# Lakonik/SSDNeRF

Hardware: NVIDIA H100
Metric: rays/sec (128^2 render) & DDIM triplanes/sec (higher is better)
Workload: dtype fp16 tensor-core UNet (fp32 accumulate), fp32 renderer

## Files before the change

### ssdnerf_b200/csrc/conv_row2.cu

```cuda
#include "common.cuh"
#include "tc_common.cuh"
#include "conv_row_epilogue.cuh"
#include "../../include/ssdnerf_b200.h"
#include <cuda_fp16.h>

namespace ssdnerf {
using namespace tc;

constexpr int kRwThreads = 384;
constexpr int kRwRowSlot = 17 * 1024;
constexpr int kRwBSlot = kRwN * 128;
constexpr int kRwRows = 6, kRwBStages = 6;
constexpr int kGnMaxC = 384;
constexpr size_t kRwSmem = (size_t)kRwRows * kRwRowSlot + (size_t)kRwBStages * kRwBSlot + 1024  + 256  +
                           256  + 512 ;

struct ConvRowParams {
    uint32_t B, H;
    const __half* x1; uint32_t C1;
    const __half* x2; uint32_t C2;
    long long xs1[3], xs2[3];
    const float2* coef;
    const float* bias;
    const __half* residual;
    __half* out;
    float* qstats;
};

template <bool GN>
__global__ void __launch_bounds__(kRwThreads, 1)
k_conv_row2(const __grid_constant__ CUtensorMap mapB, const ConvRowParams p) {
    extern __shared__ uint8_t smem_raw[];
    uint8_t* smem = reinterpret_cast<uint8_t*>(((uintptr_t)smem_raw + 1023) & ~(uintptr_t)1023);
    uint8_t* sR = smem;
    uint8_t* sB = smem + kRwRows * kRwRowSlot;
    uint64_t* fullR = reinterpret_cast<uint64_t*>(sB + kRwBStages * kRwBSlot);
    uint64_t* emptyR = fullR + kRwRows;
    uint64_t* fullB = emptyR + kRwRows;
    uint64_t* emptyB = fullB + kRwBStages;
    float* qacc = reinterpret_cast<float*>(reinterpret_cast<uint8_t*>(fullR) + 256);
    float* sbias = qacc + 64;

    const int warp = threadIdx.x >> 5, lane = threadIdx.x & 31, wg = warp >> 2;
    const uint32_t tiles_per_img = p.H / 2, total_tiles = p.B * tiles_per_img;
    const uint32_t kc1 = p.C1 / 64, KC = (p.C1 + p.C2) / 64;
    const uint32_t tile0 = blockIdx.x, tstep = gridDim.x;
    const uint32_t my_tiles = tile0 < total_tiles ? (total_tiles - tile0 + tstep - 1) / tstep : 0;

    if (threadIdx.x == 0) {
        prefetch_tmap(&mapB);
        for (int i = 0; i < kRwRows; ++i) { mbar_init(&fullR[i], 4); mbar_init(&emptyR[i], 8); }
        for (int i = 0; i < kRwBStages; ++i) { mbar_init(&fullB[i], 1); mbar_init(&emptyB[i], 8); }
        fence_mbar_init();
    }
    for (int i = threadIdx.x; i < 64; i += kRwThreads) qacc[i] = 0.0f;
    for (int i = threadIdx.x; i < kRwN; i += kRwThreads) sbias[i] = p.bias ? __ldg(p.bias + i) : 0.0f;
    __syncthreads();
    pdl_trigger();
    pdl_wait();

    if (wg == 2) {
        setmaxnreg_dec<120>();
        const uint32_t lt = threadIdx.x - 256u;
        const uint32_t c8 = lt & 7u, p0 = lt >> 3;
        const uint32_t C = p.C1 + p.C2;
        uint32_t idx = 0;
        for (uint32_t tile = tile0; tile < total_tiles; tile += tstep) {
            const uint32_t b = tile / tiles_per_img, y0 = (tile - b * tiles_per_img) * 2;
            for (uint32_t j = 0; j < KC; ++j) {
                const bool first = j < kc1;
                const __half* src = first ? p.x1 : p.x2;
                const long long xs0 = first ? p.xs1[0] : p.xs2[0], xs1 = first ? p.xs1[1] : p.xs2[1], xs2 = first ? p.xs1[2] : p.xs2[2];
                const uint32_t cl = (first ? j : j - kc1) * 64u + c8 * 8u;
                float ca[8], cb[8];
                if (GN) {
                    const float4* cp = reinterpret_cast<const float4*>(p.coef + (size_t)b * C + j * 64u + c8 * 8u);
#pragma unroll
                    for (int k = 0; k < 4; ++k) {
                        const float4 t = __ldg(cp + k);
                        ca[2 * k] = 0.5f * t.x; cb[2 * k] = 0.5f * t.y; ca[2 * k + 1] = 0.5f * t.z; cb[2 * k + 1] = 0.5f * t.w;
                    }
                }
                for (uint32_t r = 0; r < 4; ++r) {
                    const int y = (int)(y0 + r) - 1;
                    const bool row_ok = y >= 0 && y < (int)p.H;
                    const __half* rowp = src + (long long)b * xs2 + (long long)(row_ok ? y : 0) * xs1 + cl;
                    uint4 v[9];
#pragma unroll
                    for (int n = 0; n < 9; ++n) {
                        const int x = (int)(p0 + 16u * n) - 1;
                        v[n] = (row_ok && (unsigned)x < (unsigned)kRwW) ? __ldg(reinterpret_cast<const uint4*>(rowp + (long long)x * xs0))
                                                                       : make_uint4(0, 0, 0, 0);
                    }
                    const uint32_t slot = idx % kRwRows;
                    mbar_wait(&emptyR[slot], ((idx / kRwRows) & 1u) ^ 1u);
                    const uint32_t dst = smem_u32(sR + slot * kRwRowSlot);
#pragma unroll
                    for (int n = 0; n < 9; ++n) {
                        const uint32_t px = p0 + 16u * n;
                        if (px >= 130u) continue;
                        uint4 o = v[n];
                        if (GN) {
                            const bool ok = row_ok && (unsigned)((int)px - 1) < (unsigned)kRwW;
                            const __half2* h = reinterpret_cast<const __half2*>(&v[n]);
                            uint32_t* ow = reinterpret_cast<uint32_t*>(&o);
#pragma unroll
                            for (int k = 0; k < 4; ++k) {
                                const float2 tt = __half22float2(h[k]);
                                const __half2 hh = __floats2half2_rn(fmaf(tt.x, ca[2 * k], cb[2 * k]), fmaf(tt.y, ca[2 * k + 1], cb[2 * k + 1]));
                                uint32_t hv = *reinterpret_cast<const uint32_t*>(&hh), tv;
                                asm("tanh.approx.f16x2 %0, %1;" : "=r"(tv) : "r"(hv));
                                const __half2 yy = __hfma2(hh, *reinterpret_cast<const __half2*>(&tv), hh);
                                ow[k] = ok ? *reinterpret_cast<const uint32_t*>(&yy) : 0u;
                            }
                        }
                        sts128(dst + px * 128u + ((c8 ^ (px & 7u)) << 4), o);
                    }
                    __syncwarp();
                    if (lane == 0) mbar_arrive(&fullR[slot]);
                    ++idx;
                }
            }
        }
    } else {
        setmaxnreg_inc<192>();
        const uint32_t a = (uint32_t)wg, wq = (uint32_t)warp & 3u, cq = (uint32_t)lane & 3u;
        const uint32_t steps_per_tile = KC * 9u, total_steps = my_tiles * steps_per_tile;
        auto issue_w = [&](uint32_t L) {
            const uint32_t s = L % kRwBStages;
            if (L >= (uint32_t)kRwBStages) mbar_wait(&emptyB[s], ((L / kRwBStages) - 1u) & 1u);
            mbar_expect_tx(&fullB[s], (uint32_t)kRwBSlot);
            const uint32_t rem = L % steps_per_tile;
            tma_load_4d(sB + s * kRwBSlot, &mapB, &fullB[s], (int)((rem / 9u) * 64u), 0, (int)(rem % 9u), 0);
        };
        if (threadIdx.x == 0)
            for (uint32_t L = 0; L < total_steps && L < (uint32_t)kRwBStages; ++L) issue_w(L);
        auto release_row = [&](uint32_t ring) { if (lane == 0) mbar_arrive(&emptyR[ring % kRwRows]); };
        uint32_t m = 0, ridx = 0;
        const uint32_t lrow = wq * 16u + ((uint32_t)lane & 15u);
        const uint32_t lk = (uint32_t)lane >> 4;
        for (uint32_t tile = tile0; tile < total_tiles; tile += tstep) {
            const uint32_t b = tile / tiles_per_img, y0 = (tile - b * tiles_per_img) * 2;
            float acc0[64], acc1[64];
#pragma unroll
            for (int i = 0; i < 64; ++i) { acc0[i] = 0.0f; acc1[i] = 0.0f; }
            for (uint32_t j = 0; j < KC; ++j) {
                const uint32_t unused = ridx + (a == 0 ? 3u : 0u);
                if (a == 1) { mbar_wait(&fullR[unused % kRwRows], (unused / kRwRows) & 1u); release_row(unused); }
                for (uint32_t ky = 0; ky < 3; ++ky) {
                    const uint32_t ring = ridx + ky + a;
                    mbar_wait(&fullR[ring % kRwRows], (ring / kRwRows) & 1u);
                    const uint32_t rowS = smem_u32(sR + (ring % kRwRows) * kRwRowSlot);
                    for (uint32_t kx = 0; kx < 3; ++kx) {
                        const uint32_t sb = m % kRwBStages;
                        uint32_t af[2][4][4];
#pragma unroll
                        for (uint32_t h = 0; h < 2; ++h) {
                            const uint32_t px = 64u * h + lrow + kx;
#pragma unroll
                            for (uint32_t k = 0; k < 4; ++k) ldmatrix_x4(rowS + px * 128u + (((2u * k + lk) ^ (px & 7u)) << 4), af[h][k]);
                        }
                        if (kx == 2) release_row(ring);
                        mbar_wait(&fullB[sb], (m / kRwBStages) & 1u);
                        const uint64_t b_desc = make_desc_sw128(smem_u32(sB + sb * kRwBSlot));
                        wgmma_fence();
                        fence_regs(acc0); fence_regs(acc1);
#pragma unroll
                        for (uint32_t k = 0; k < 4; ++k) {
                            wgmma_rs_n128(acc0, af[0][k], b_desc + 2 * k, 1u);
                            wgmma_rs_n128(acc1, af[1][k], b_desc + 2 * k, 1u);
                        }
                        wgmma_commit();
                        wgmma_wait<0>();
                        fence_regs(acc0); fence_regs(acc1);
                        if (lane == 0) mbar_arrive(&emptyB[sb]);
                        if (threadIdx.x == 0 && m >= 1 && m - 1 + kRwBStages < total_steps) issue_w(m - 1 + kRwBStages);
                        ++m;
                    }
                }
                if (a == 0) { mbar_wait(&fullR[unused % kRwRows], (unused / kRwRows) & 1u); release_row(unused); }
                ridx += 4;
            }
            const size_t pix0 = ((size_t)b * p.H + y0 + a) * kRwW;
#pragma unroll
            for (int i = 0; i < 16; ++i) {
                const uint32_t ch = 8u * i + 2u * cq;
                const float b0 = sbias[ch], b1 = sbias[ch + 1];
                float su = 0.0f, sq = 0.0f;
#pragma unroll
                for (int h = 0; h < 2; ++h) {
#pragma unroll
                    for (int hh = 0; hh < 2; ++hh) {
                        const size_t o = (pix0 + 64u * h + wq * 16u + ((uint32_t)lane >> 2) + 8u * hh) * kRwN + ch;
                        float v0 = (h ? acc1 : acc0)[4 * i + 2 * hh] + b0, v1 = (h ? acc1 : acc0)[4 * i + 2 * hh + 1] + b1;
                        if (p.residual) { const float2 r = __half22float2(*reinterpret_cast<const __half2*>(p.residual + o)); v0 += r.x; v1 += r.y; }
                        *reinterpret_cast<__half2*>(p.out + o) = __floats2half2_rn(v0, v1);
                        su += v0 + v1; sq = fmaf(v0, v0, fmaf(v1, v1, sq));
                    }
                }
                if (p.qstats) {
                    frag_quad_reduce(su, sq);
                    if ((lane & ~2) == 0) { float* qa = qacc + (2 * i + (lane >> 1)) * 2; atomicAdd(qa, su); atomicAdd(qa + 1, sq); }
                }
            }
            if (p.qstats) {
                asm volatile("bar.sync 1, 256;" ::: "memory");
                if (threadIdx.x < 64) {
                    const float val = qacc[threadIdx.x];
                    if (val != 0.0f) atomicAdd(p.qstats + (size_t)b * 64 + threadIdx.x, val);
                    qacc[threadIdx.x] = 0.0f;
                }
                asm volatile("bar.sync 1, 256;" ::: "memory");
            }
        }
    }
    __syncthreads();
}

__global__ void k_gn_coef(const float* __restrict__ q1, uint32_t C1, const float* __restrict__ q2, uint32_t C2, uint32_t HW,
                          const float* __restrict__ gamma, const float* __restrict__ beta, const float* __restrict__ scale_shift,
                          long long ss_batch_stride, float eps, float2* __restrict__ coef) {
    pdl_trigger();
    pdl_wait();
    __shared__ float2 s_mr[32];
    const uint32_t b = blockIdx.x, C = C1 + C2, cpg = C / 32u;
    const float inv_n = 1.0f / ((float)HW * (float)cpg);
    if (threadIdx.x < 32u) {
        const uint32_t q1n = C1 / 4, q2n = C2 / 4, nq = cpg / 4;
        float sm = 0.0f, sq = 0.0f;
        for (uint32_t i = 0; i < nq; ++i) {
            const uint32_t qi = threadIdx.x * nq + i;
            const float2 t = __ldg(reinterpret_cast<const float2*>(qi < q1n ? q1 + ((size_t)b * q1n + qi) * 2 : q2 + ((size_t)b * q2n + (qi - q1n)) * 2));
            sm += t.x; sq += t.y;
        }
        const float mean = sm * inv_n;
        s_mr[threadIdx.x] = make_float2(mean, rsqrtf(fmaxf(sq * inv_n - mean * mean, 0.0f) + eps));
    }
    __syncthreads();
    const float* ss = scale_shift ? scale_shift + (size_t)b * ss_batch_stride : nullptr;
    for (uint32_t c = threadIdx.x; c < C; c += blockDim.x) {
        const float2 mr = s_mr[c / cpg];
        const float ak = mr.y * __ldg(gamma + c);
        const float bk = __ldg(beta + c) - mr.x * ak;
        const float sc = ss ? 1.0f + __ldg(ss + c) : 1.0f, sh = ss ? __ldg(ss + C + c) : 0.0f;
        coef[(size_t)b * C + c] = make_float2(ak * sc, fmaf(bk, sc, sh));
    }
}

int make_map_4d_box(CUtensorMap* m, const void* base, uint64_t K, uint64_t e1, uint64_t e2, uint64_t e3, uint64_t s1, uint64_t s2, uint64_t s3,
                    uint32_t x1, uint32_t x2, uint32_t x3);

template <bool GN>
static int launch_row2(const CUtensorMap& mB, const ConvRowParams& p, int sms, cudaStream_t stream) {
    static DeviceOnce attr;
    if (attr.first()) {
        SSDNERF_CUDA_OK(cudaFuncSetAttribute(k_conv_row2<GN>, cudaFuncAttributeMaxDynamicSharedMemorySize, (int)kRwSmem));
    }
    const uint32_t total = p.B * (p.H / 2);
    SSDNERF_CUDA_OK(launch_pdl(k_conv_row2<GN>, dim3(total < (uint32_t)sms ? total : (uint32_t)sms), dim3(kRwThreads), kRwSmem, stream, mB, p));
    SSDNERF_LAUNCH_OK();
    return 0;
}

int conv_row2_launch(const ssdnerf_gemm_args* a, int sms, cudaStream_t stream) {
    if (((uintptr_t)a->a1 & 15u) || ((a->a1_strides[0] | a->a1_strides[1] | a->a1_strides[2]) & 15u) ||
        (a->a2 && (((uintptr_t)a->a2 & 15u) || ((a->a2_strides[0] | a->a2_strides[1] | a->a2_strides[2]) & 15u))) ||
        ((uintptr_t)a->out & 3u) || ((uintptr_t)a->residual & 3u))
        return set_error_msg(SSDNERF_ERR_ARG, "gemm: row-pair convolution needs 16-byte aligned inputs and strides, 4-byte aligned output / residual");
    ConvRowParams p{};
    p.B = a->d3; p.H = a->d2;
    p.x1 = (const __half*)a->a1; p.C1 = a->k1;
    p.x2 = (const __half*)a->a2; p.C2 = a->a2 ? a->k2 : 0;
    for (int i = 0; i < 3; ++i) { p.xs1[i] = (long long)(a->a1_strides[i] / 2); p.xs2[i] = a->a2 ? (long long)(a->a2_strides[i] / 2) : 0; }
    p.bias = a->bias_n; p.residual = (const __half*)a->residual; p.out = (__half*)a->out; p.qstats = a->qstats;
    const uint64_t ktot = (uint64_t)a->k1 + (a->a2 ? a->k2 : 0);
    CUtensorMap mB;
    if (int e = make_map_4d_box(&mB, a->b, ktot, a->n_rows_b ? a->n_rows_b : a->n, a->bx2 ? a->bx2 : 1, a->bx3 ? a->bx3 : 1, a->b_strides[0],
                                a->b_strides[1], a->b_strides[2], kRwN, 1, 1)) return e;
    return launch_row2<false>(mB, p, sms, stream);
}

}

using namespace ssdnerf;

extern "C" int ssdnerf_conv3x3_gn_f16(const ssdnerf_conv_gn_args* a, void* stream_) {
    cudaStream_t stream = (cudaStream_t)stream_;
    if (!a || !a->x1 || !a->q1 || !a->gamma || !a->beta || !a->w || !a->out || !a->coef_workspace)
        return set_error_msg(SSDNERF_ERR_ARG, "conv3x3_gn: x1, q1, gamma, beta, w, out and coef_workspace are required");
    if (a->B == 0 || a->H == 0) return 0;
    if (a->H % 2) return set_error_msg(SSDNERF_ERR_ARG, "conv3x3_gn: H must be even (tiles are row pairs)");
    if (a->C1 == 0 || a->C1 % 64 || a->C2 % 64 || (a->x2 && !a->q2)) return set_error_msg(SSDNERF_ERR_ARG, "conv3x3_gn: channel counts must be multiples of 64; x2 needs q2");
    const uint32_t C = a->C1 + (a->x2 ? a->C2 : 0);
    if (C > (uint32_t)kGnMaxC || (C / 32) % 4) return set_error_msg(SSDNERF_ERR_ARG, "conv3x3_gn: at most 384 input channels, channels per group a multiple of 4");
    if (a->w_rows < 128) return set_error_msg(SSDNERF_ERR_ARG, "conv3x3_gn: packed weight needs >= 128 rows per tap");
    if (((uintptr_t)a->x1 | (uintptr_t)a->x2 | (uintptr_t)a->out | (uintptr_t)a->residual | (uintptr_t)a->w | (uintptr_t)a->coef_workspace) & 15u)
        return set_error_msg(SSDNERF_ERR_ARG, "conv3x3_gn: tensors must be 16-byte aligned");
    ConvRowParams p{};
    p.B = a->B; p.H = a->H; p.x1 = (const __half*)a->x1; p.C1 = a->C1; p.x2 = (const __half*)a->x2; p.C2 = a->x2 ? a->C2 : 0;
    p.xs1[0] = p.C1; p.xs1[1] = (long long)kRwW * p.C1; p.xs1[2] = (long long)p.H * kRwW * p.C1;
    p.xs2[0] = p.C2; p.xs2[1] = (long long)kRwW * p.C2; p.xs2[2] = (long long)p.H * kRwW * p.C2;
    p.coef = (const float2*)a->coef_workspace; p.bias = a->bias; p.residual = (const __half*)a->residual; p.out = (__half*)a->out; p.qstats = a->qstats;
    int dev = 0, sms = 0;
    SSDNERF_CUDA_OK(cudaGetDevice(&dev));
    SSDNERF_CUDA_OK(cudaDeviceGetAttribute(&sms, cudaDevAttrMultiProcessorCount, dev));
    SSDNERF_CUDA_OK(launch_pdl(k_gn_coef, dim3(a->B), dim3(128), 0, stream, a->q1, a->C1, a->x2 ? a->q2 : (const float*)nullptr, p.C2, a->H * 128u,
                               a->gamma, a->beta, a->scale_shift, a->ss_batch_stride, a->eps, (float2*)a->coef_workspace));
    SSDNERF_LAUNCH_OK();
    CUtensorMap mB;
    if (int e = make_map_4d_box(&mB, a->w, C, a->w_rows, 9, 1, (uint64_t)C * 2, (uint64_t)a->w_rows * C * 2, (uint64_t)9 * a->w_rows * C * 2,
                                kRwN, 1, 1)) return e;
    return launch_row2<true>(mB, p, sms, stream);
}
```

### ssdnerf_b200/csrc/conv_row_epilogue.cuh

```cuda
#pragma once
#include "common.cuh"

namespace ssdnerf {

constexpr int kRwW = 128, kRwN = 128;

__device__ __forceinline__ void frag_quad_reduce(float& su, float& sq) {
    su += __shfl_xor_sync(0xffffffffu, su, 1); sq += __shfl_xor_sync(0xffffffffu, sq, 1);
#pragma unroll
    for (int m = 4; m <= 16; m <<= 1) { su += __shfl_xor_sync(0xffffffffu, su, m); sq += __shfl_xor_sync(0xffffffffu, sq, m); }
}

}
```

### ssdnerf_b200/csrc/gemm_tc.cu

```cuda
#include "common.cuh"
#include "tc_common.cuh"
#include "conv_row_epilogue.cuh"
#include "../../include/ssdnerf_b200.h"
#include <cuda_fp16.h>
#include <cstdio>

namespace ssdnerf {
using namespace tc;

constexpr int kGemmThreads = 384;
constexpr int kMaxBiasN = 2048;
constexpr int kBM = 128, kBK = 64;
constexpr int kABytes = kBM * kBK * 2;

struct GemmParams {
    uint32_t b1, b2, b3;
    uint32_t d1, d2, d3;
    uint32_t T1, T2, T3;
    uint32_t tiles_n;
    uint32_t taps;
    int8_t tap_ox[9], tap_oy[9];
    uint32_t a_stride;
    uint32_t kc1, kc2;
    uint32_t n_valid;
    uint32_t b_batched;
    uint32_t vec2;
    float alpha;
    const float* bias_n;
    const __half* residual;
    void* out;
    uint32_t out_f32;
    long long so1, so2, so3;
    float* qstats;
    uint32_t stats_hw;
    unsigned long long* prof;
};

template <int BN, int CL>
struct GemmCfg {
    static constexpr int kBBytes = BN * kBK * 2;
    static constexpr int kBoxRowsB = BN / CL;
    static constexpr int kStageBytes = kABytes + kBBytes;
    static constexpr int kStages = (192 * 1024 / kStageBytes) > 8 ? 8 : (192 * 1024 / kStageBytes);
    static constexpr size_t kSmem = (size_t)kStages * kStageBytes + 1024  + 256  + 1024  +
                                    kMaxBiasN * 4 ;
};

template <int BN, int CL>
__global__ void __launch_bounds__(kGemmThreads, 1)
k_gemm_tc(const __grid_constant__ CUtensorMap mapA1, const __grid_constant__ CUtensorMap mapA2,
          const __grid_constant__ CUtensorMap mapB, const GemmParams p) {
    using Cfg = GemmCfg<BN, CL>;
    extern __shared__ uint8_t smem_raw[];
    uint8_t* smem = reinterpret_cast<uint8_t*>(((uintptr_t)smem_raw + 1023) & ~(uintptr_t)1023);
    uint8_t* sA = smem;
    uint8_t* sB = smem + Cfg::kStages * kABytes;
    uint64_t* full = reinterpret_cast<uint64_t*>(smem + Cfg::kStages * Cfg::kStageBytes);
    uint64_t* empty = full + Cfg::kStages;
    float* qacc = reinterpret_cast<float*>(smem + Cfg::kStages * Cfg::kStageBytes + 256);
    float* sbias = qacc + 256;

    const int warp = threadIdx.x >> 5, lane = threadIdx.x & 31, wg = warp >> 2;
    const uint32_t tiles_m = p.T1 * p.T2 * p.T3;
    const uint32_t sup_m = (tiles_m + CL - 1) / CL;
    const uint32_t total_tiles = sup_m * p.tiles_n;
    const uint32_t iters = p.taps * (p.kc1 + p.kc2);
    const uint32_t crank = (CL > 1) ? cluster_ctarank() : 0u;
    const uint32_t tile0 = (CL > 1) ? cluster_id_x() : blockIdx.x;
    const uint32_t tile_step = (CL > 1) ? num_clusters_x() : gridDim.x;
    constexpr uint16_t kMask = (uint16_t)((1u << CL) - 1u);

    if (threadIdx.x == 0) {
        prefetch_tmap(&mapA1); prefetch_tmap(&mapA2); prefetch_tmap(&mapB);
        for (int i = 0; i < Cfg::kStages; ++i) { mbar_init(&full[i], 1); mbar_init(&empty[i], 8 * CL); }
        fence_mbar_init();
    }
    for (int i = threadIdx.x; i < BN; i += kGemmThreads) qacc[i] = 0.0f;
    if (p.bias_n) for (uint32_t i = threadIdx.x; i < p.n_valid; i += kGemmThreads) sbias[i] = __ldg(p.bias_n + i);
    __syncthreads();
    if (CL > 1) cluster_sync_all();
    pdl_trigger();
    pdl_wait();

    if (wg == 0) {
        setmaxnreg_dec<40>();
        if (threadIdx.x == 0) {
            uint32_t stage = 0, phase = 0;
            long long pw = 0; const long long pt0 = clock64();
            for (uint32_t tile = tile0; tile < total_tiles; tile += tile_step) {
                const uint32_t m_tile = (tile % sup_m) * CL + crank, n_tile = tile / sup_m;
                const uint32_t t1 = m_tile % p.T1, t2 = (m_tile / p.T1) % p.T2, t3 = m_tile / (p.T1 * p.T2);
                for (uint32_t tap = 0; tap < p.taps; ++tap) {
                    const int ox = p.tap_ox[tap], oy = p.tap_oy[tap];
                    for (uint32_t j = 0; j < p.kc1 + p.kc2; ++j) {
                        if (p.prof) { const long long c = clock64(); mbar_wait(&empty[stage], phase ^ 1); pw += clock64() - c; }
                        else mbar_wait(&empty[stage], phase ^ 1);
                        const bool first = j < p.kc1;
                        const int ak = (int)((first ? j : j - p.kc1) * kBK), a1 = (int)(t1 * p.b1 * p.a_stride) + ox, a2 = (int)(t2 * p.b2 * p.a_stride) + oy, a3 = (int)(t3 * p.b3);
                        mbar_expect_tx(&full[stage], (uint32_t)Cfg::kStageBytes);
                        tma_load_4d(sA + stage * kABytes, first ? &mapA1 : &mapA2, &full[stage], ak, a1, a2, a3);
                        if (CL == 1) {
                            tma_load_4d(sB + stage * Cfg::kBBytes, &mapB, &full[stage], (int)(j * kBK), (int)(n_tile * BN),
                                        p.b_batched ? (int)t2 : (int)tap, p.b_batched ? (int)t3 : 0);
                        } else {
                            tma_load_4d_mc(sB + stage * Cfg::kBBytes + crank * Cfg::kBoxRowsB * 128, &mapB, &full[stage], (int)(j * kBK),
                                           (int)(n_tile * BN + crank * Cfg::kBoxRowsB), (int)tap, 0, kMask);
                        }
                        if (++stage == Cfg::kStages) { stage = 0; phase ^= 1; }
                    }
                }
            }
            if (p.prof) { atomicAdd(p.prof + 0, (unsigned long long)pw); atomicAdd(p.prof + 1, (unsigned long long)(clock64() - pt0)); }
        }
    } else {
        setmaxnreg_inc<232>();
        const uint32_t cw = (uint32_t)wg - 1u;
        const uint32_t wq = (uint32_t)warp & 3u;
        const uint32_t rbase = cw * 64u + wq * 16u + ((uint32_t)lane >> 2);
        const uint32_t cq = (uint32_t)lane & 3u;
        uint32_t stage = 0, phase = 0;
        long long wf = 0; const long long ct0 = clock64();
        float acc[BN / 2];
        auto release = [&](uint32_t s) {
            if (lane == 0) {
                if (CL == 1) mbar_arrive(&empty[s]);
                else for (uint32_t r = 0; r < (uint32_t)CL; ++r) mbar_arrive_cluster(mapa_u32(smem_u32(&empty[s]), r));
            }
        };
        for (uint32_t tile = tile0; tile < total_tiles; tile += tile_step) {
            const uint32_t m_tile = (tile % sup_m) * CL + crank, n_tile = tile / sup_m;
            const uint32_t t1 = m_tile % p.T1, t2 = (m_tile / p.T1) % p.T2, t3 = m_tile / (p.T1 * p.T2);
#pragma unroll
            for (int i = 0; i < BN / 2; ++i) acc[i] = 0.0f;
            uint32_t prev = 0;
            for (uint32_t it = 0; it < iters; ++it) {
                if (p.prof && cw == 0) { const long long c = clock64(); mbar_wait(&full[stage], phase); wf += clock64() - c; }
                else mbar_wait(&full[stage], phase);
                const uint64_t a_desc = make_desc_sw128(smem_u32(sA + stage * kABytes + cw * 64 * 128));
                const uint64_t b_desc = make_desc_sw128(smem_u32(sB + stage * Cfg::kBBytes));
                wgmma_fence();
                fence_regs(acc);
#pragma unroll
                for (uint32_t k = 0; k < kBK / 16; ++k) {
                    if constexpr (BN == 256) wgmma_ss_n256(acc, a_desc + 2 * k, b_desc + 2 * k, 1u);
                    else if constexpr (BN == 128) wgmma_ss_n128(acc, a_desc + 2 * k, b_desc + 2 * k, 1u);
                    else wgmma_ss_n64(acc, a_desc + 2 * k, b_desc + 2 * k, 1u);
                }
                wgmma_commit();
                fence_regs(acc);
                wgmma_wait<1>();
                if (it > 0) release(prev);
                prev = stage;
                if (++stage == Cfg::kStages) { stage = 0; phase ^= 1; }
            }
            wgmma_wait<0>();
            fence_regs(acc);
            if (iters > 0) release(prev);

            long long off[2]; bool rok[2];
#pragma unroll
            for (int h = 0; h < 2; ++h) {
                const uint32_t row = rbase + 8u * h;
                const uint32_t i1 = row % p.b1, i2 = (row / p.b1) % p.b2, i3 = row / (p.b1 * p.b2);
                const uint32_t g1 = t1 * p.b1 + i1, g2 = t2 * p.b2 + i2, g3 = t3 * p.b3 + i3;
                rok[h] = m_tile < tiles_m && g1 < p.d1 && g2 < p.d2 && g3 < p.d3;
                off[h] = (long long)g1 * p.so1 + (long long)g2 * p.so2 + (long long)g3 * p.so3 + (long long)n_tile * BN;
            }
            uint32_t slot = 0, img0 = 0;
            if (p.qstats) {
                const uint32_t r0 = cw * 64u;
                const uint32_t j1 = r0 % p.b1, j3 = r0 / (p.b1 * p.b2);
                img0 = p.stats_hw ? (t1 * p.b1) / p.stats_hw : t3 * p.b3;
                slot = ((p.stats_hw ? (t1 * p.b1 + j1) / p.stats_hw : t3 * p.b3 + j3) - img0) & 1u;
            }
#pragma unroll
            for (int i = 0; i < BN / 8; ++i) {
                const uint32_t c0 = 8u * i + 2u * cq;
                const uint32_t ncol = n_tile * BN + c0;
                const bool okc0 = ncol < p.n_valid, okc1 = ncol + 1 < p.n_valid;
                float su = 0.0f, sq = 0.0f;
#pragma unroll
                for (int h = 0; h < 2; ++h) {
                    float v0 = acc[4 * i + 2 * h] * p.alpha, v1 = acc[4 * i + 2 * h + 1] * p.alpha;
                    if (!rok[h] || !okc0) continue;
                    if (p.bias_n) { v0 += sbias[ncol]; if (okc1) v1 += sbias[ncol + 1]; }
                    const long long o = off[h] + c0;
                    if (p.residual) {
                        if (p.vec2 && okc1) {
                            const float2 r = __half22float2(*reinterpret_cast<const __half2*>(p.residual + o));
                            v0 += r.x; v1 += r.y;
                        } else {
                            v0 += __half2float(p.residual[o]);
                            if (okc1) v1 += __half2float(p.residual[o + 1]);
                        }
                    }
                    if (p.out_f32) {
                        float* op = reinterpret_cast<float*>(p.out) + o;
                        if (p.vec2 && okc1) *reinterpret_cast<float2*>(op) = make_float2(v0, v1);
                        else { op[0] = v0; if (okc1) op[1] = v1; }
                    } else {
                        __half* op = reinterpret_cast<__half*>(p.out) + o;
                        if (p.vec2 && okc1) *reinterpret_cast<__half2*>(op) = __floats2half2_rn(v0, v1);
                        else { op[0] = __float2half_rn(v0); if (okc1) op[1] = __float2half_rn(v1); }
                    }
                    if (!okc1) v1 = 0.0f;
                    su += v0 + v1; sq = fmaf(v0, v0, fmaf(v1, v1, sq));
                }
                if (p.qstats) {
                    frag_quad_reduce(su, sq);
                    if ((lane & ~2) == 0) {
                        float* qa = qacc + (slot * (BN / 4) + 2 * i + (lane >> 1)) * 2;
                        atomicAdd(qa, su); atomicAdd(qa + 1, sq);
                    }
                }
            }
            if (p.qstats) {
                asm volatile("bar.sync 1, 256;" ::: "memory");
                const uint32_t et = threadIdx.x - 128;
                const uint32_t nq = p.n_valid / 4;
                for (uint32_t i = et; i < (uint32_t)BN; i += 256) {
                    const float val = qacc[i];
                    const uint32_t sl = i / (BN / 2), qd = (i % (BN / 2)) >> 1, st = i & 1u;
                    const uint32_t gq = n_tile * (BN / 4) + qd;
                    if (val != 0.0f && gq < nq) atomicAdd(p.qstats + ((size_t)(img0 + sl) * nq + gq) * 2 + st, val);
                    qacc[i] = 0.0f;
                }
                asm volatile("bar.sync 1, 256;" ::: "memory");
            }
        }
        if (p.prof && threadIdx.x == 128) { atomicAdd(p.prof + 2, (unsigned long long)wf); atomicAdd(p.prof + 4, (unsigned long long)(clock64() - ct0)); }
    }
    __syncthreads();
    if (CL > 1) cluster_sync_all();
}

typedef CUresult (*PFN_encodeTiled)(CUtensorMap*, CUtensorMapDataType, cuuint32_t, void*, const cuuint64_t*, const cuuint64_t*,
                                    const cuuint32_t*, const cuuint32_t*, CUtensorMapInterleave, CUtensorMapSwizzle,
                                    CUtensorMapL2promotion, CUtensorMapFloatOOBfill);

static PFN_encodeTiled get_encode() {
    static PFN_encodeTiled fn = nullptr;
    if (!fn) {
        void* p = nullptr;
        cudaDriverEntryPointQueryResult qres;
        if (cudaGetDriverEntryPoint("cuTensorMapEncodeTiled", &p, cudaEnableDefault, &qres) != cudaSuccess || !p) return nullptr;
        fn = (PFN_encodeTiled)p;
    }
    return fn;
}

static int make_map_4d(CUtensorMap* m, const void* base, uint64_t K, uint64_t e1, uint64_t e2, uint64_t e3, uint64_t s1, uint64_t s2,
                       uint64_t s3, uint32_t x1, uint32_t x2, uint32_t x3, uint32_t trav = 1) {
    PFN_encodeTiled enc = get_encode();
    if (!enc) return set_error_msg(SSDNERF_ERR_CUDA, "cuTensorMapEncodeTiled entry point not found");
    if (((uintptr_t)base & 15u) || (s1 & 15u) || (s2 & 15u) || (s3 & 15u))
        return set_error_msg(SSDNERF_ERR_ARG, "gemm: TMA operands need 16-byte aligned base and strides");
    cuuint64_t dims[4] = {K, e1, e2, e3};
    cuuint64_t strides[3] = {s1, s2, s3};
    cuuint32_t box[4] = {64, x1 * trav, x2 * trav, x3};
    cuuint32_t estr[4] = {1, trav, trav, 1};
    const CUresult r = enc(m, CU_TENSOR_MAP_DATA_TYPE_FLOAT16, 4, const_cast<void*>(base), dims, strides, box, estr,
                           CU_TENSOR_MAP_INTERLEAVE_NONE, CU_TENSOR_MAP_SWIZZLE_128B, CU_TENSOR_MAP_L2_PROMOTION_L2_256B,
                           CU_TENSOR_MAP_FLOAT_OOB_FILL_NONE);
    if (r != CUDA_SUCCESS) {
        char buf[200];
        snprintf(buf, sizeof(buf), "cuTensorMapEncodeTiled failed (%d): dims {%llu,%llu,%llu,%llu} box {64,%u,%u,%u}", (int)r,
                 (unsigned long long)K, (unsigned long long)e1, (unsigned long long)e2, (unsigned long long)e3, x1, x2, x3);
        return set_error_msg(SSDNERF_ERR_CUDA, buf);
    }
    return 0;
}

int make_map_4d_box(CUtensorMap* m, const void* base, uint64_t K, uint64_t e1, uint64_t e2, uint64_t e3, uint64_t s1, uint64_t s2, uint64_t s3,
                    uint32_t x1, uint32_t x2, uint32_t x3) {
    return make_map_4d(m, base, K, e1, e2, e3, s1, s2, s3, x1, x2, x3);
}
int conv_row2_launch(const ssdnerf_gemm_args* a, int sms, cudaStream_t stream);

template <int BN, int CL>
static int launch_gemm(const CUtensorMap& mA1, const CUtensorMap& mA2, const CUtensorMap& mB, const GemmParams& p, int sms,
                       cudaStream_t stream) {
    using Cfg = GemmCfg<BN, CL>;
    static DeviceOnce attr;
    if (attr.first()) {
        SSDNERF_CUDA_OK(cudaFuncSetAttribute(k_gemm_tc<BN, CL>, cudaFuncAttributeMaxDynamicSharedMemorySize, (int)Cfg::kSmem));
    }
    const uint32_t tiles_m = p.T1 * p.T2 * p.T3;
    const uint32_t total = ((tiles_m + CL - 1) / CL) * p.tiles_n;
    cudaLaunchConfig_t cfg{};
    cfg.blockDim = dim3(kGemmThreads);
    cfg.dynamicSmemBytes = Cfg::kSmem;
    cfg.stream = stream;
    cudaLaunchAttribute at[2];
    at[0].id = cudaLaunchAttributeClusterDimension;
    at[0].val.clusterDim.x = CL; at[0].val.clusterDim.y = 1; at[0].val.clusterDim.z = 1;
    at[1].id = cudaLaunchAttributeProgrammaticStreamSerialization;
    at[1].val.programmaticStreamSerializationAllowed = pdl_enabled() ? 1 : 0;
    cfg.attrs = at; cfg.numAttrs = 2;
    static int max_clusters_dev[64] = {};
    int& max_clusters_cached = max_clusters_dev[current_device()];
    if (!max_clusters_cached) {
        max_clusters_cached = sms / CL;
        if (CL > 1) {
            cfg.gridDim = dim3((uint32_t)(sms / CL) * CL);
            int n = 0;
            cfg.numAttrs = 1;
            if (cudaOccupancyMaxActiveClusters(&n, k_gemm_tc<BN, CL>, &cfg) == cudaSuccess && n > 0 && n < max_clusters_cached) max_clusters_cached = n;
            cfg.numAttrs = 2;
            (void)cudaGetLastError();
        }
    }
    const uint32_t max_clusters = (uint32_t)max_clusters_cached;
    const uint32_t clusters = total < max_clusters ? total : max_clusters;
    cfg.gridDim = dim3(clusters * CL);
    SSDNERF_CUDA_OK(cudaLaunchKernelEx(&cfg, k_gemm_tc<BN, CL>, mA1, mA2, mB, p));
    SSDNERF_LAUNCH_OK();
    return 0;
}

}

using namespace ssdnerf;

extern "C" int ssdnerf_gemm_f16(const ssdnerf_gemm_args* a, void* stream_) {
    cudaStream_t stream = (cudaStream_t)stream_;
    if (!a || !a->a1 || !a->b || !a->out) return set_error_msg(SSDNERF_ERR_ARG, "gemm: a1, b and out are required");
    if (a->k1 == 0 || a->k1 % 64 || a->k2 % 64) return set_error_msg(SSDNERF_ERR_ARG, "gemm: K extents must be multiples of 64");
    if (a->b1 * a->b2 * a->b3 != 128) return set_error_msg(SSDNERF_ERR_ARG, "gemm: b1*b2*b3 must be 128");
    if (a->taps < 1 || a->taps > 9) return set_error_msg(SSDNERF_ERR_ARG, "gemm: taps must be in [1, 9]");
    if (a->taps != 1 && a->taps != 9 && !a->tap_offsets) return set_error_msg(SSDNERF_ERR_ARG, "gemm: taps other than 1 / 9 need tap_offsets");
    if (a->taps > 1 && a->b_batched) return set_error_msg(SSDNERF_ERR_ARG, "gemm: conv taps and batched B are exclusive");
    if (a->a_stride > 2) return set_error_msg(SSDNERF_ERR_ARG, "gemm: a_stride must be 0 / 1 / 2");
    const uint32_t a_stride = a->a_stride == 2 ? 2u : 1u;
    if (a_stride == 2 && (a->b1 * 2 > 256 || a->b2 * 2 > 256)) return set_error_msg(SSDNERF_ERR_ARG, "gemm: stride-2 boxes exceed the 256-element TMA limit");
    if (a->n == 0 || a->d1 == 0 || a->d2 == 0 || a->d3 == 0) return 0;
    int dev = 0, sms = 0;
    SSDNERF_CUDA_OK(cudaGetDevice(&dev));
    SSDNERF_CUDA_OK(cudaDeviceGetAttribute(&sms, cudaDevAttrMultiProcessorCount, dev));
    if (a->algo != 1 && a->taps == 9 && !a->tap_offsets && a_stride == 1 && a->d1 == 128 && a->b1 == 128 && a->b2 == 1 && a->b3 == 1 && a->n == 128 && !a->out_f32 && !a->b_batched &&
        (a->d2 % 2) == 0 && a->alpha == 1.0f && (a->bn == 0 || a->bn == 128) && a->cluster <= 1 && a->so1 == 128 && a->so2 == 128 * 128 &&
        a->so3 == (long long)a->d2 * 128 * 128 && (!a->qstats || a->stats_hw == 0) && (a->n_rows_b == 0 || a->n_rows_b >= 128))
        return ssdnerf::conv_row2_launch(a, sms, stream);
    if (a->algo == 2) return set_error_msg(SSDNERF_ERR_ARG, "gemm: algo 2 (row-pair convolution) needs taps 9, 128-pixel rows, 128 output channels, fp16 output");
    int bn = (int)a->bn;
    if (!bn) {
        const uint32_t tiles_m = div_up(a->d1, a->b1) * div_up(a->d2, a->b2) * div_up(a->d3, a->b3);
        double best = 1e30;
        const int cand[3] = {256, 128, 64};
        const double eff[3] = {1.0, 0.80, 0.50};
        for (int i = 0; i < 3; ++i) {
            if (cand[i] > 64 && (uint32_t)cand[i] / 2 >= a->n) continue;
            const uint32_t tiles = tiles_m * div_up(a->n, (uint32_t)cand[i]);
            const double t = (double)div_up(tiles, (uint32_t)sms) * cand[i] / eff[i];
            if (t < best) { best = t; bn = cand[i]; }
        }
    }
    if (bn != 64 && bn != 128 && bn != 256) return set_error_msg(SSDNERF_ERR_ARG, "gemm: bn must be 64, 128 or 256");

    GemmParams p{};
    p.b1 = a->b1; p.b2 = a->b2; p.b3 = a->b3; p.d1 = a->d1; p.d2 = a->d2; p.d3 = a->d3;
    p.T1 = div_up(a->d1, a->b1); p.T2 = div_up(a->d2, a->b2); p.T3 = div_up(a->d3, a->b3);
    p.tiles_n = div_up(a->n, (uint32_t)bn);
    p.a_stride = a_stride;
    for (uint32_t t = 0; t < 9; ++t) {
        if (a->tap_offsets) { p.tap_ox[t] = a->tap_offsets[2 * t]; p.tap_oy[t] = a->tap_offsets[2 * t + 1]; }
        else if (a->taps == 9) { p.tap_ox[t] = (int8_t)((int)(t % 3) - 1); p.tap_oy[t] = (int8_t)((int)(t / 3) - 1); }
        else { p.tap_ox[t] = 0; p.tap_oy[t] = 0; }
    }
    p.taps = a->taps; p.kc1 = a->k1 / 64; p.kc2 = a->a2 ? a->k2 / 64 : 0; p.n_valid = a->n; p.b_batched = a->b_batched;
    p.alpha = a->alpha; p.bias_n = a->bias_n; p.residual = (const __half*)a->residual; p.out = a->out; p.out_f32 = a->out_f32;
    p.so1 = a->so1; p.so2 = a->so2; p.so3 = a->so3;
    p.qstats = a->qstats; p.stats_hw = a->stats_hw; p.prof = (unsigned long long*)a->debug_cycles;
    const uintptr_t pair_align = a->out_f32 ? 8u : 4u;
    p.vec2 = ((a->so1 | a->so2 | a->so3) & 1) == 0 && ((uintptr_t)a->out % pair_align) == 0 && ((uintptr_t)a->residual & 3u) == 0;
    if (a->bias_n && a->n > (uint32_t)kMaxBiasN) return set_error_msg(SSDNERF_ERR_ARG, "gemm: bias vectors longer than 2048 are not supported");
    if (a->qstats && (a->n % 4)) return set_error_msg(SSDNERF_ERR_ARG, "gemm: quad statistics need n % 4 == 0");
    if (a->qstats && !a->stats_hw && a->b3 > 2) return set_error_msg(SSDNERF_ERR_ARG, "gemm: fused quad statistics cover at most 2 images per 128-row tile (b3 <= 2)");
    if (a->qstats && a->stats_hw && (a->stats_hw % 64)) return set_error_msg(SSDNERF_ERR_ARG, "gemm: stats_hw must be a multiple of 64");
    const uint64_t ktot = (uint64_t)a->k1 + (a->a2 ? a->k2 : 0);

    CUtensorMap mA1, mA2, mB;
    const uint64_t e1 = (uint64_t)a->d1 * a_stride, e2 = (uint64_t)a->d2 * a_stride;
    if (int e = make_map_4d(&mA1, a->a1, a->k1, e1, e2, a->d3, a->a1_strides[0], a->a1_strides[1], a->a1_strides[2], a->b1, a->b2, a->b3, a_stride)) return e;
    if (a->a2) {
        if (int e = make_map_4d(&mA2, a->a2, a->k2, e1, e2, a->d3, a->a2_strides[0], a->a2_strides[1], a->a2_strides[2], a->b1, a->b2, a->b3, a_stride)) return e;
    } else {
        mA2 = mA1;
    }
    int cl = 1;
    if ((a->cluster == 2 || a->cluster == 4 || a->cluster == 8) && !a->b_batched && bn >= 128) cl = (int)a->cluster;
    if (int e = make_map_4d(&mB, a->b, ktot, a->n_rows_b ? a->n_rows_b : a->n, a->bx2 ? a->bx2 : 1, a->bx3 ? a->bx3 : 1, a->b_strides[0],
                            a->b_strides[1], a->b_strides[2], (uint32_t)(bn / cl), 1, 1)) return e;

    if (bn == 256) {
        if (cl == 8) return launch_gemm<256, 8>(mA1, mA2, mB, p, sms, stream);
        if (cl == 4) return launch_gemm<256, 4>(mA1, mA2, mB, p, sms, stream);
        return cl == 2 ? launch_gemm<256, 2>(mA1, mA2, mB, p, sms, stream) : launch_gemm<256, 1>(mA1, mA2, mB, p, sms, stream);
    }
    if (bn == 128) {
        if (cl == 8) return launch_gemm<128, 8>(mA1, mA2, mB, p, sms, stream);
        if (cl == 4) return launch_gemm<128, 4>(mA1, mA2, mB, p, sms, stream);
        return cl == 2 ? launch_gemm<128, 2>(mA1, mA2, mB, p, sms, stream) : launch_gemm<128, 1>(mA1, mA2, mB, p, sms, stream);
    }
    return launch_gemm<64, 1>(mA1, mA2, mB, p, sms, stream);
}
```

### ssdnerf_b200/csrc/tc_common.cuh

```cuda
#pragma once
#include <cuda.h>
#include <cuda_runtime.h>
#include <stdint.h>

namespace ssdnerf {
namespace tc {

__device__ __forceinline__ uint32_t smem_u32(const void* p) { return (uint32_t)__cvta_generic_to_shared(p); }

__device__ __forceinline__ void sts128(uint32_t addr, const uint4& v) {
    asm volatile("st.shared.v4.b32 [%0], {%1, %2, %3, %4};" ::"r"(addr), "r"(v.x), "r"(v.y), "r"(v.z), "r"(v.w) : "memory");
}

__device__ __forceinline__ void mbar_init(uint64_t* bar, uint32_t count) {
    asm volatile("mbarrier.init.shared::cta.b64 [%0], %1;" ::"r"(smem_u32(bar)), "r"(count));
}
__device__ __forceinline__ void fence_mbar_init() { asm volatile("fence.mbarrier_init.release.cluster;" ::: "memory"); }
__device__ __forceinline__ void mbar_arrive(uint64_t* bar) {
    asm volatile("mbarrier.arrive.shared::cta.b64 _, [%0];" ::"r"(smem_u32(bar)) : "memory");
}
__device__ __forceinline__ void mbar_wait(uint64_t* bar, uint32_t parity) {
    uint32_t spins = 0, ok = 0;
    while (!ok) {
        asm volatile(
            "{\n\t.reg .pred p;\n\t"
            "mbarrier.try_wait.parity.acquire.cluster.shared::cta.b64 p, [%1], %2;\n\t"
            "selp.b32 %0, 1, 0, p;\n\t}"
            : "=r"(ok) : "r"(smem_u32(bar)), "r"(parity) : "memory");
        if (!ok && ++spins > 200000000u) { asm volatile("trap;"); }
    }
}
__device__ __forceinline__ void mbar_expect_tx(uint64_t* bar, uint32_t bytes) {
    asm volatile("mbarrier.arrive.expect_tx.shared::cta.b64 _, [%0], %1;" ::"r"(smem_u32(bar)), "r"(bytes) : "memory");
}

__device__ __forceinline__ uint32_t cluster_ctarank() { uint32_t r; asm volatile("mov.u32 %0, %%cluster_ctarank;" : "=r"(r)); return r; }
__device__ __forceinline__ uint32_t cluster_id_x() { uint32_t r; asm volatile("mov.u32 %0, %%clusterid.x;" : "=r"(r)); return r; }
__device__ __forceinline__ uint32_t num_clusters_x() { uint32_t r; asm volatile("mov.u32 %0, %%nclusterid.x;" : "=r"(r)); return r; }
__device__ __forceinline__ void cluster_sync_all() {
    asm volatile("barrier.cluster.arrive.release.aligned;" ::: "memory");
    asm volatile("barrier.cluster.wait.acquire.aligned;" ::: "memory");
}
__device__ __forceinline__ uint32_t mapa_u32(uint32_t smem_addr, uint32_t rank) {
    uint32_t r;
    asm volatile("mapa.shared::cluster.u32 %0, %1, %2;" : "=r"(r) : "r"(smem_addr), "r"(rank));
    return r;
}
__device__ __forceinline__ void mbar_arrive_cluster(uint32_t cluster_addr) {
    asm volatile("mbarrier.arrive.release.cluster.shared::cluster.b64 _, [%0];" ::"r"(cluster_addr) : "memory");
}

__device__ __forceinline__ void prefetch_tmap(const CUtensorMap* m) {
    asm volatile("prefetch.tensormap [%0];" ::"l"(reinterpret_cast<uint64_t>(m)) : "memory");
}
__device__ __forceinline__ void tma_load_4d(void* dst, const CUtensorMap* m, uint64_t* bar, int c0, int c1, int c2, int c3) {
    asm volatile(
        "cp.async.bulk.tensor.4d.shared::cluster.global.mbarrier::complete_tx::bytes [%0], [%1, {%3, %4, %5, %6}], [%2];"
        ::"r"(smem_u32(dst)), "l"(reinterpret_cast<uint64_t>(m)), "r"(smem_u32(bar)), "r"(c0), "r"(c1), "r"(c2), "r"(c3)
        : "memory");
}
__device__ __forceinline__ void tma_load_4d_mc(void* dst, const CUtensorMap* m, uint64_t* bar, int c0, int c1, int c2, int c3, uint16_t cta_mask) {
    asm volatile(
        "cp.async.bulk.tensor.4d.shared::cluster.global.mbarrier::complete_tx::bytes.multicast::cluster [%0], [%1, {%4, %5, %6, %7}], [%2], %3;"
        ::"r"(smem_u32(dst)), "l"(reinterpret_cast<uint64_t>(m)), "r"(smem_u32(bar)), "h"(cta_mask), "r"(c0), "r"(c1), "r"(c2), "r"(c3)
        : "memory");
}
__device__ __forceinline__ void fence_proxy_async_smem() { asm volatile("fence.proxy.async.shared::cta;" ::: "memory"); }

template <int N> __device__ __forceinline__ void setmaxnreg_inc() { asm volatile("setmaxnreg.inc.sync.aligned.u32 %0;" ::"n"(N)); }
template <int N> __device__ __forceinline__ void setmaxnreg_dec() { asm volatile("setmaxnreg.dec.sync.aligned.u32 %0;" ::"n"(N)); }

__device__ __forceinline__ uint64_t make_desc_sw128(uint32_t smem_addr) {
    uint64_t d = 0;
    d |= (uint64_t)((smem_addr >> 4) & 0x3FFFu);
    d |= (uint64_t)1 << 16;
    d |= (uint64_t)(1024u >> 4) << 32;
    d |= (uint64_t)1 << 62;
    return d;
}
__device__ __forceinline__ void wgmma_fence() { asm volatile("wgmma.fence.sync.aligned;" ::: "memory"); }
__device__ __forceinline__ void wgmma_commit() { asm volatile("wgmma.commit_group.sync.aligned;" ::: "memory"); }
template <int N> __device__ __forceinline__ void wgmma_wait() { asm volatile("wgmma.wait_group.sync.aligned %0;" ::"n"(N) : "memory"); }
template <int R> __device__ __forceinline__ void fence_regs(float (&d)[R]) {
#pragma unroll
    for (int i = 0; i < R; ++i) asm volatile("" : "+f"(d[i])::"memory");
}

__device__ __forceinline__ void ldmatrix_x4(uint32_t addr, uint32_t (&r)[4]) {
    asm volatile("ldmatrix.sync.aligned.m8n8.x4.shared.b16 {%0, %1, %2, %3}, [%4];"
                 : "=r"(r[0]), "=r"(r[1]), "=r"(r[2]), "=r"(r[3]) : "r"(addr) : "memory");
}

__device__ __forceinline__ void wgmma_ss_n64(float (&d)[32], uint64_t a_desc, uint64_t b_desc, uint32_t accumulate) {
    asm volatile(
        "{\n\t.reg .pred p;\n\t"
        "setp.ne.b32 p, %34, 0;\n\t"
        "wgmma.mma_async.sync.aligned.m64n64k16.f32.f16.f16 "
        "{%0, %1, %2, %3, %4, %5, %6, %7, %8, %9, %10, %11, %12, %13, %14, %15, %16, %17, %18, %19, %20, %21, %22, %23, %24, %25, %26, %27, %28, %29, %30, %31}, %32, %33, p, 1, 1, 0, 0;\n\t}"
        : "+f"(d[0]), "+f"(d[1]), "+f"(d[2]), "+f"(d[3]), "+f"(d[4]), "+f"(d[5]), "+f"(d[6]), "+f"(d[7]), "+f"(d[8]), "+f"(d[9]), "+f"(d[10]), "+f"(d[11]), "+f"(d[12]), "+f"(d[13]), "+f"(d[14]), "+f"(d[15]), "+f"(d[16]), "+f"(d[17]), "+f"(d[18]), "+f"(d[19]), "+f"(d[20]), "+f"(d[21]), "+f"(d[22]), "+f"(d[23]), "+f"(d[24]), "+f"(d[25]), "+f"(d[26]), "+f"(d[27]), "+f"(d[28]), "+f"(d[29]), "+f"(d[30]), "+f"(d[31])
        : "l"(a_desc), "l"(b_desc), "r"(accumulate));
}
__device__ __forceinline__ void wgmma_ss_n128(float (&d)[64], uint64_t a_desc, uint64_t b_desc, uint32_t accumulate) {
    asm volatile(
        "{\n\t.reg .pred p;\n\t"
        "setp.ne.b32 p, %66, 0;\n\t"
        "wgmma.mma_async.sync.aligned.m64n128k16.f32.f16.f16 "
        "{%0, %1, %2, %3, %4, %5, %6, %7, %8, %9, %10, %11, %12, %13, %14, %15, %16, %17, %18, %19, %20, %21, %22, %23, %24, %25, %26, %27, %28, %29, %30, %31, %32, %33, %34, %35, %36, %37, %38, %39, %40, %41, %42, %43, %44, %45, %46, %47, %48, %49, %50, %51, %52, %53, %54, %55, %56, %57, %58, %59, %60, %61, %62, %63}, %64, %65, p, 1, 1, 0, 0;\n\t}"
        : "+f"(d[0]), "+f"(d[1]), "+f"(d[2]), "+f"(d[3]), "+f"(d[4]), "+f"(d[5]), "+f"(d[6]), "+f"(d[7]), "+f"(d[8]), "+f"(d[9]), "+f"(d[10]), "+f"(d[11]), "+f"(d[12]), "+f"(d[13]), "+f"(d[14]), "+f"(d[15]), "+f"(d[16]), "+f"(d[17]), "+f"(d[18]), "+f"(d[19]), "+f"(d[20]), "+f"(d[21]), "+f"(d[22]), "+f"(d[23]), "+f"(d[24]), "+f"(d[25]), "+f"(d[26]), "+f"(d[27]), "+f"(d[28]), "+f"(d[29]), "+f"(d[30]), "+f"(d[31]), "+f"(d[32]), "+f"(d[33]), "+f"(d[34]), "+f"(d[35]), "+f"(d[36]), "+f"(d[37]), "+f"(d[38]), "+f"(d[39]), "+f"(d[40]), "+f"(d[41]), "+f"(d[42]), "+f"(d[43]), "+f"(d[44]), "+f"(d[45]), "+f"(d[46]), "+f"(d[47]), "+f"(d[48]), "+f"(d[49]), "+f"(d[50]), "+f"(d[51]), "+f"(d[52]), "+f"(d[53]), "+f"(d[54]), "+f"(d[55]), "+f"(d[56]), "+f"(d[57]), "+f"(d[58]), "+f"(d[59]), "+f"(d[60]), "+f"(d[61]), "+f"(d[62]), "+f"(d[63])
        : "l"(a_desc), "l"(b_desc), "r"(accumulate));
}
__device__ __forceinline__ void wgmma_rs_n128(float (&d)[64], const uint32_t (&a)[4], uint64_t b_desc, uint32_t accumulate) {
    asm volatile(
        "{\n\t.reg .pred p;\n\t"
        "setp.ne.b32 p, %69, 0;\n\t"
        "wgmma.mma_async.sync.aligned.m64n128k16.f32.f16.f16 "
        "{%0, %1, %2, %3, %4, %5, %6, %7, %8, %9, %10, %11, %12, %13, %14, %15, %16, %17, %18, %19, %20, %21, %22, %23, %24, %25, %26, %27, %28, %29, %30, %31, %32, %33, %34, %35, %36, %37, %38, %39, %40, %41, %42, %43, %44, %45, %46, %47, %48, %49, %50, %51, %52, %53, %54, %55, %56, %57, %58, %59, %60, %61, %62, %63}, {%64, %65, %66, %67}, %68, p, 1, 1, 0;\n\t}"
        : "+f"(d[0]), "+f"(d[1]), "+f"(d[2]), "+f"(d[3]), "+f"(d[4]), "+f"(d[5]), "+f"(d[6]), "+f"(d[7]), "+f"(d[8]), "+f"(d[9]), "+f"(d[10]), "+f"(d[11]), "+f"(d[12]), "+f"(d[13]), "+f"(d[14]), "+f"(d[15]), "+f"(d[16]), "+f"(d[17]), "+f"(d[18]), "+f"(d[19]), "+f"(d[20]), "+f"(d[21]), "+f"(d[22]), "+f"(d[23]), "+f"(d[24]), "+f"(d[25]), "+f"(d[26]), "+f"(d[27]), "+f"(d[28]), "+f"(d[29]), "+f"(d[30]), "+f"(d[31]), "+f"(d[32]), "+f"(d[33]), "+f"(d[34]), "+f"(d[35]), "+f"(d[36]), "+f"(d[37]), "+f"(d[38]), "+f"(d[39]), "+f"(d[40]), "+f"(d[41]), "+f"(d[42]), "+f"(d[43]), "+f"(d[44]), "+f"(d[45]), "+f"(d[46]), "+f"(d[47]), "+f"(d[48]), "+f"(d[49]), "+f"(d[50]), "+f"(d[51]), "+f"(d[52]), "+f"(d[53]), "+f"(d[54]), "+f"(d[55]), "+f"(d[56]), "+f"(d[57]), "+f"(d[58]), "+f"(d[59]), "+f"(d[60]), "+f"(d[61]), "+f"(d[62]), "+f"(d[63])
        : "r"(a[0]), "r"(a[1]), "r"(a[2]), "r"(a[3]), "l"(b_desc), "r"(accumulate));
}
__device__ __forceinline__ void wgmma_ss_n256(float (&d)[128], uint64_t a_desc, uint64_t b_desc, uint32_t accumulate) {
    asm volatile(
        "{\n\t.reg .pred p;\n\t"
        "setp.ne.b32 p, %130, 0;\n\t"
        "wgmma.mma_async.sync.aligned.m64n256k16.f32.f16.f16 "
        "{%0, %1, %2, %3, %4, %5, %6, %7, %8, %9, %10, %11, %12, %13, %14, %15, %16, %17, %18, %19, %20, %21, %22, %23, %24, %25, %26, %27, %28, %29, %30, %31, %32, %33, %34, %35, %36, %37, %38, %39, %40, %41, %42, %43, %44, %45, %46, %47, %48, %49, %50, %51, %52, %53, %54, %55, %56, %57, %58, %59, %60, %61, %62, %63, %64, %65, %66, %67, %68, %69, %70, %71, %72, %73, %74, %75, %76, %77, %78, %79, %80, %81, %82, %83, %84, %85, %86, %87, %88, %89, %90, %91, %92, %93, %94, %95, %96, %97, %98, %99, %100, %101, %102, %103, %104, %105, %106, %107, %108, %109, %110, %111, %112, %113, %114, %115, %116, %117, %118, %119, %120, %121, %122, %123, %124, %125, %126, %127}, %128, %129, p, 1, 1, 0, 0;\n\t}"
        : "+f"(d[0]), "+f"(d[1]), "+f"(d[2]), "+f"(d[3]), "+f"(d[4]), "+f"(d[5]), "+f"(d[6]), "+f"(d[7]), "+f"(d[8]), "+f"(d[9]), "+f"(d[10]), "+f"(d[11]), "+f"(d[12]), "+f"(d[13]), "+f"(d[14]), "+f"(d[15]), "+f"(d[16]), "+f"(d[17]), "+f"(d[18]), "+f"(d[19]), "+f"(d[20]), "+f"(d[21]), "+f"(d[22]), "+f"(d[23]), "+f"(d[24]), "+f"(d[25]), "+f"(d[26]), "+f"(d[27]), "+f"(d[28]), "+f"(d[29]), "+f"(d[30]), "+f"(d[31]), "+f"(d[32]), "+f"(d[33]), "+f"(d[34]), "+f"(d[35]), "+f"(d[36]), "+f"(d[37]), "+f"(d[38]), "+f"(d[39]), "+f"(d[40]), "+f"(d[41]), "+f"(d[42]), "+f"(d[43]), "+f"(d[44]), "+f"(d[45]), "+f"(d[46]), "+f"(d[47]), "+f"(d[48]), "+f"(d[49]), "+f"(d[50]), "+f"(d[51]), "+f"(d[52]), "+f"(d[53]), "+f"(d[54]), "+f"(d[55]), "+f"(d[56]), "+f"(d[57]), "+f"(d[58]), "+f"(d[59]), "+f"(d[60]), "+f"(d[61]), "+f"(d[62]), "+f"(d[63]), "+f"(d[64]), "+f"(d[65]), "+f"(d[66]), "+f"(d[67]), "+f"(d[68]), "+f"(d[69]), "+f"(d[70]), "+f"(d[71]), "+f"(d[72]), "+f"(d[73]), "+f"(d[74]), "+f"(d[75]), "+f"(d[76]), "+f"(d[77]), "+f"(d[78]), "+f"(d[79]), "+f"(d[80]), "+f"(d[81]), "+f"(d[82]), "+f"(d[83]), "+f"(d[84]), "+f"(d[85]), "+f"(d[86]), "+f"(d[87]), "+f"(d[88]), "+f"(d[89]), "+f"(d[90]), "+f"(d[91]), "+f"(d[92]), "+f"(d[93]), "+f"(d[94]), "+f"(d[95]), "+f"(d[96]), "+f"(d[97]), "+f"(d[98]), "+f"(d[99]), "+f"(d[100]), "+f"(d[101]), "+f"(d[102]), "+f"(d[103]), "+f"(d[104]), "+f"(d[105]), "+f"(d[106]), "+f"(d[107]), "+f"(d[108]), "+f"(d[109]), "+f"(d[110]), "+f"(d[111]), "+f"(d[112]), "+f"(d[113]), "+f"(d[114]), "+f"(d[115]), "+f"(d[116]), "+f"(d[117]), "+f"(d[118]), "+f"(d[119]), "+f"(d[120]), "+f"(d[121]), "+f"(d[122]), "+f"(d[123]), "+f"(d[124]), "+f"(d[125]), "+f"(d[126]), "+f"(d[127])
        : "l"(a_desc), "l"(b_desc), "r"(accumulate));
}

}
}
```

Measured before the change: 80.09 million.

## Generalize row-pair conv kernel to 64-wide rows and TMA-load activations

Templates the row-pair 3x3 convolution kernel on row width and output channels, which lets 64-pixel rows with 256 output channels use it via a new register-sourced m64n256 wgmma. In the non-GroupNorm path, activation rows now come in through TMA from a single producer thread instead of manual global loads and swizzled stores. A dedicated warp also issues the weight loads. The MMA loop double-buffers fragment loads with wgmma_wait<1> so ldmatrix overlaps the tensor-core work. The cost is higher register pressure (setmaxnreg raised to 232) and more complex barrier accounting.

```diff
diff --git a/ssdnerf_b200/csrc/conv_row2.cu b/ssdnerf_b200/csrc/conv_row2.cu
--- a/ssdnerf_b200/csrc/conv_row2.cu
+++ b/ssdnerf_b200/csrc/conv_row2.cu
@@ -8,12 +8,21 @@
 using namespace tc;
 
 constexpr int kRwThreads = 384;
-constexpr int kRwRowSlot = 17 * 1024;
-constexpr int kRwBSlot = kRwN * 128;
-constexpr int kRwRows = 6, kRwBStages = 6;
 constexpr int kGnMaxC = 384;
-constexpr size_t kRwSmem = (size_t)kRwRows * kRwRowSlot + (size_t)kRwBStages * kRwBSlot + 1024  + 256  +
-                           256  + 512 ;
+
+template <int W, int N>
+struct RowCfg {
+    static constexpr int kHalves = W / 64;
+    static constexpr int kRowBytes = (W + 2) * 128;
+    static constexpr int kRowSlot = (kRowBytes + 1023) / 1024 * 1024;
+    static constexpr int kBSlot = N * 128;
+    static constexpr int kRows = 6;
+    static constexpr int kBStages = W == 128 ? 7 : 5;
+    static constexpr size_t kSmem = (size_t)kRows * kRowSlot + (size_t)kBStages * kBSlot + 1024  + 256  +
+                                    N * 2  + N * 4 ;
+    static_assert(kSmem <= 227 * 1024, "row kernel shared memory");
+    static_assert(2 * (kRows + kBStages) * 8 <= 256, "row kernel barriers");
+};
 
 struct ConvRowParams {
     uint32_t B, H;
@@ -27,81 +36,121 @@
     float* qstats;
 };
 
-template <bool GN>
+template <int N>
+__device__ __forceinline__ void wgmma_rs_row(float (&d)[N / 2], const uint32_t (&a)[4], uint64_t b_desc) {
+    if constexpr (N == 256) wgmma_rs_n256(d, a, b_desc, 1u);
+    else wgmma_rs_n128(d, a, b_desc, 1u);
+}
+
+template <bool GN, int W, int N>
 __global__ void __launch_bounds__(kRwThreads, 1)
-k_conv_row2(const __grid_constant__ CUtensorMap mapB, const ConvRowParams p) {
+k_conv_row2(const __grid_constant__ CUtensorMap mapB, const __grid_constant__ CUtensorMap mapX1, const __grid_constant__ CUtensorMap mapX2,
+            const ConvRowParams p) {
+    using Cfg = RowCfg<W, N>;
+    static_assert(!GN || (W == 128 && N == 128), "the GroupNorm-fused loader covers 128-pixel rows, 128 output channels");
+    constexpr int kH = Cfg::kHalves, kRows = Cfg::kRows, kS = Cfg::kBStages;
     extern __shared__ uint8_t smem_raw[];
     uint8_t* smem = reinterpret_cast<uint8_t*>(((uintptr_t)smem_raw + 1023) & ~(uintptr_t)1023);
     uint8_t* sR = smem;
-    uint8_t* sB = smem + kRwRows * kRwRowSlot;
-    uint64_t* fullR = reinterpret_cast<uint64_t*>(sB + kRwBStages * kRwBSlot);
-    uint64_t* emptyR = fullR + kRwRows;
-    uint64_t* fullB = emptyR + kRwRows;
-    uint64_t* emptyB = fullB + kRwBStages;
+    uint8_t* sB = smem + kRows * Cfg::kRowSlot;
+    uint64_t* fullR = reinterpret_cast<uint64_t*>(sB + kS * Cfg::kBSlot);
+    uint64_t* emptyR = fullR + kRows;
+    uint64_t* fullB = emptyR + kRows;
+    uint64_t* emptyB = fullB + kS;
     float* qacc = reinterpret_cast<float*>(reinterpret_cast<uint8_t*>(fullR) + 256);
-    float* sbias = qacc + 64;
+    float* sbias = qacc + N / 2;
 
     const int warp = threadIdx.x >> 5, lane = threadIdx.x & 31, wg = warp >> 2;
     const uint32_t tiles_per_img = p.H / 2, total_tiles = p.B * tiles_per_img;
     const uint32_t kc1 = p.C1 / 64, KC = (p.C1 + p.C2) / 64;
     const uint32_t tile0 = blockIdx.x, tstep = gridDim.x;
     const uint32_t my_tiles = tile0 < total_tiles ? (total_tiles - tile0 + tstep - 1) / tstep : 0;
+    const uint32_t steps_per_tile = KC * 9u, total_steps = my_tiles * steps_per_tile;
 
     if (threadIdx.x == 0) {
         prefetch_tmap(&mapB);
-        for (int i = 0; i < kRwRows; ++i) { mbar_init(&fullR[i], 4); mbar_init(&emptyR[i], 8); }
-        for (int i = 0; i < kRwBStages; ++i) { mbar_init(&fullB[i], 1); mbar_init(&emptyB[i], 8); }
+        for (int i = 0; i < kRows; ++i) { mbar_init(&fullR[i], GN ? 4 : 1); mbar_init(&emptyR[i], 8); }
+        for (int i = 0; i < kS; ++i) { mbar_init(&fullB[i], 1); mbar_init(&emptyB[i], 8); }
         fence_mbar_init();
     }
-    for (int i = threadIdx.x; i < 64; i += kRwThreads) qacc[i] = 0.0f;
-    for (int i = threadIdx.x; i < kRwN; i += kRwThreads) sbias[i] = p.bias ? __ldg(p.bias + i) : 0.0f;
+    for (int i = threadIdx.x; i < N / 2; i += kRwThreads) qacc[i] = 0.0f;
+    for (int i = threadIdx.x; i < N; i += kRwThreads) sbias[i] = p.bias ? __ldg(p.bias + i) : 0.0f;
     __syncthreads();
     pdl_trigger();
     pdl_wait();
 
+    auto issue_w = [&](uint32_t L) {
+        const uint32_t s = L % kS;
+        if (L >= (uint32_t)kS) mbar_wait(&emptyB[s], ((L / kS) - 1u) & 1u);
+        mbar_expect_tx(&fullB[s], (uint32_t)Cfg::kBSlot);
+        const uint32_t rem = L % steps_per_tile;
+        tma_load_4d(sB + s * Cfg::kBSlot, &mapB, &fullB[s], (int)((rem / 9u) * 64u), 0, (int)(rem % 9u), 0);
+    };
+
     if (wg == 2) {
-        setmaxnreg_dec<120>();
-        const uint32_t lt = threadIdx.x - 256u;
-        const uint32_t c8 = lt & 7u, p0 = lt >> 3;
-        const uint32_t C = p.C1 + p.C2;
-        uint32_t idx = 0;
-        for (uint32_t tile = tile0; tile < total_tiles; tile += tstep) {
-            const uint32_t b = tile / tiles_per_img, y0 = (tile - b * tiles_per_img) * 2;
-            for (uint32_t j = 0; j < KC; ++j) {
-                const bool first = j < kc1;
-                const __half* src = first ? p.x1 : p.x2;
-                const long long xs0 = first ? p.xs1[0] : p.xs2[0], xs1 = first ? p.xs1[1] : p.xs2[1], xs2 = first ? p.xs1[2] : p.xs2[2];
-                const uint32_t cl = (first ? j : j - kc1) * 64u + c8 * 8u;
-                float ca[8], cb[8];
-                if (GN) {
-                    const float4* cp = reinterpret_cast<const float4*>(p.coef + (size_t)b * C + j * 64u + c8 * 8u);
-#pragma unroll
-                    for (int k = 0; k < 4; ++k) {
-                        const float4 t = __ldg(cp + k);
-                        ca[2 * k] = 0.5f * t.x; cb[2 * k] = 0.5f * t.y; ca[2 * k + 1] = 0.5f * t.z; cb[2 * k + 1] = 0.5f * t.w;
+        if constexpr (!GN) {
+            setmaxnreg_dec<40>();
+            if (warp == 8 && lane == 0) {
+                prefetch_tmap(&mapX1); prefetch_tmap(&mapX2);
+                uint32_t idx = 0;
+                for (uint32_t tile = tile0; tile < total_tiles; tile += tstep) {
+                    const uint32_t b = tile / tiles_per_img, y0 = (tile - b * tiles_per_img) * 2;
+                    for (uint32_t j = 0; j < KC; ++j) {
+                        const bool first = j < kc1;
+                        const int c = (int)((first ? j : j - kc1) * 64u);
+                        for (uint32_t r = 0; r < 4; ++r, ++idx) {
+                            const uint32_t slot = idx % kRows;
+                            mbar_wait(&emptyR[slot], ((idx / kRows) & 1u) ^ 1u);
+                            mbar_expect_tx(&fullR[slot], (uint32_t)Cfg::kRowBytes);
+                            tma_load_4d(sR + slot * Cfg::kRowSlot, first ? &mapX1 : &mapX2, &fullR[slot], c, -1, (int)(y0 + r) - 1, (int)b);
+                        }
                     }
                 }
-                for (uint32_t r = 0; r < 4; ++r) {
-                    const int y = (int)(y0 + r) - 1;
-                    const bool row_ok = y >= 0 && y < (int)p.H;
-                    const __half* rowp = src + (long long)b * xs2 + (long long)(row_ok ? y : 0) * xs1 + cl;
-                    uint4 v[9];
-#pragma unroll
-                    for (int n = 0; n < 9; ++n) {
-                        const int x = (int)(p0 + 16u * n) - 1;
-                        v[n] = (row_ok && (unsigned)x < (unsigned)kRwW) ? __ldg(reinterpret_cast<const uint4*>(rowp + (long long)x * xs0))
-                                                                       : make_uint4(0, 0, 0, 0);
+            } else if (warp == 9 && lane == 0) {
+                for (uint32_t L = 0; L < total_steps; ++L) issue_w(L);
+            }
+        } else {
+            setmaxnreg_dec<120>();
+            const uint32_t lt = threadIdx.x - 256u;
+            const uint32_t c8 = lt & 7u, p0 = lt >> 3;
+            const uint32_t C = p.C1 + p.C2;
+            uint32_t idx = 0;
+            for (uint32_t tile = tile0; tile < total_tiles; tile += tstep) {
+                const uint32_t b = tile / tiles_per_img, y0 = (tile - b * tiles_per_img) * 2;
+                for (uint32_t j = 0; j < KC; ++j) {
+                    const bool first = j < kc1;
+                    const __half* src = first ? p.x1 : p.x2;
+                    const long long xs0 = first ? p.xs1[0] : p.xs2[0], xs1 = first ? p.xs1[1] : p.xs2[1], xs2 = first ? p.xs1[2] : p.xs2[2];
+                    const uint32_t cl = (first ? j : j - kc1) * 64u + c8 * 8u;
+                    float ca[8], cb[8];
+                    {
+                        const float4* cp = reinterpret_cast<const float4*>(p.coef + (size_t)b * C + j * 64u + c8 * 8u);
+#pragma unroll
+                        for (int k = 0; k < 4; ++k) {
+                            const float4 t = __ldg(cp + k);
+                            ca[2 * k] = 0.5f * t.x; cb[2 * k] = 0.5f * t.y; ca[2 * k + 1] = 0.5f * t.z; cb[2 * k + 1] = 0.5f * t.w;
+                        }
                     }
-                    const uint32_t slot = idx % kRwRows;
-                    mbar_wait(&emptyR[slot], ((idx / kRwRows) & 1u) ^ 1u);
-                    const uint32_t dst = smem_u32(sR + slot * kRwRowSlot);
-#pragma unroll
-                    for (int n = 0; n < 9; ++n) {
-                        const uint32_t px = p0 + 16u * n;
-                        if (px >= 130u) continue;
-                        uint4 o = v[n];
-                        if (GN) {
-                            const bool ok = row_ok && (unsigned)((int)px - 1) < (unsigned)kRwW;
+                    for (uint32_t r = 0; r < 4; ++r) {
+                        const int y = (int)(y0 + r) - 1;
+                        const bool row_ok = y >= 0 && y < (int)p.H;
+                        const __half* rowp = src + (long long)b * xs2 + (long long)(row_ok ? y : 0) * xs1 + cl;
+                        uint4 v[9];
+#pragma unroll
+                        for (int n = 0; n < 9; ++n) {
+                            const int x = (int)(p0 + 16u * n) - 1;
+                            v[n] = (row_ok && (unsigned)x < (unsigned)W) ? __ldg(reinterpret_cast<const uint4*>(rowp + (long long)x * xs0))
+                                                                         : make_uint4(0, 0, 0, 0);
+                        }
+                        const uint32_t slot = idx % kRows;
+                        mbar_wait(&emptyR[slot], ((idx / kRows) & 1u) ^ 1u);
+                        const uint32_t dst = smem_u32(sR + slot * Cfg::kRowSlot);
+#pragma unroll
+                        for (int n = 0; n < 9; ++n) {
+                            const uint32_t px = p0 + 16u * n;
+                            if (px >= (uint32_t)(W + 2)) continue;
+                            uint4 o = v[n];
+                            const bool ok = row_ok && (unsigned)((int)px - 1) < (unsigned)W;
                             const __half2* h = reinterpret_cast<const __half2*>(&v[n]);
                             uint32_t* ow = reinterpret_cast<uint32_t*>(&o);
 #pragma unroll
@@ -113,101 +162,142 @@
                                 const __half2 yy = __hfma2(hh, *reinterpret_cast<const __half2*>(&tv), hh);
                                 ow[k] = ok ? *reinterpret_cast<const uint32_t*>(&yy) : 0u;
                             }
+                            sts128(dst + px * 128u + ((c8 ^ (px & 7u)) << 4), o);
                         }
-                        sts128(dst + px * 128u + ((c8 ^ (px & 7u)) << 4), o);
+                        __syncwarp();
+                        if (lane == 0) mbar_arrive(&fullR[slot]);
+                        ++idx;
                     }
-                    __syncwarp();
-                    if (lane == 0) mbar_arrive(&fullR[slot]);
-                    ++idx;
                 }
             }
         }
     } else {
-        setmaxnreg_inc<192>();
+        if constexpr (GN) setmaxnreg_inc<192>();
+        else setmaxnreg_inc<232>();
         const uint32_t a = (uint32_t)wg, wq = (uint32_t)warp & 3u, cq = (uint32_t)lane & 3u;
-        const uint32_t steps_per_tile = KC * 9u, total_steps = my_tiles * steps_per_tile;
-        auto issue_w = [&](uint32_t L) {
-            const uint32_t s = L % kRwBStages;
-            if (L >= (uint32_t)kRwBStages) mbar_wait(&emptyB[s], ((L / kRwBStages) - 1u) & 1u);
-            mbar_expect_tx(&fullB[s], (uint32_t)kRwBSlot);
-            const uint32_t rem = L % steps_per_tile;
-            tma_load_4d(sB + s * kRwBSlot, &mapB, &fullB[s], (int)((rem / 9u) * 64u), 0, (int)(rem % 9u), 0);
-        };
-        if (threadIdx.x == 0)
-            for (uint32_t L = 0; L < total_steps && L < (uint32_t)kRwBStages; ++L) issue_w(L);
-        auto release_row = [&](uint32_t ring) { if (lane == 0) mbar_arrive(&emptyR[ring % kRwRows]); };
-        uint32_t m = 0, ridx = 0;
+        if (GN && threadIdx.x == 0)
+            for (uint32_t L = 0; L < total_steps && L < (uint32_t)kS; ++L) issue_w(L);
+        auto release_row = [&](uint32_t ring) { if (lane == 0) mbar_arrive(&emptyR[ring % kRows]); };
+        auto release_w = [&](uint32_t L) { if (lane == 0) mbar_arrive(&emptyB[L % kS]); };
         const uint32_t lrow = wq * 16u + ((uint32_t)lane & 15u);
         const uint32_t lk = (uint32_t)lane >> 4;
+        uint32_t m = 0;
+        uint32_t ridx = 0, ky = 0, kx = 0;
+        uint32_t done_row = 0;
+        float acc[kH][N / 2];
+        uint32_t af0[kH][4][4], af1[kH][4][4];
+
+        auto load_frags = [&](uint32_t (&f)[kH][4][4]) {
+            if (a == 1 && ky == 0 && kx == 0) { mbar_wait(&fullR[ridx % kRows], (ridx / kRows) & 1u); release_row(ridx); }
+            const uint32_t ring = ridx + ky + a;
+            if (kx == 0) mbar_wait(&fullR[ring % kRows], (ring / kRows) & 1u);
+            const uint32_t rowS = smem_u32(sR + (ring % kRows) * Cfg::kRowSlot);
+#pragma unroll
+            for (uint32_t h = 0; h < (uint32_t)kH; ++h) {
+                const uint32_t px = 64u * h + lrow + kx;
+#pragma unroll
+                for (uint32_t k = 0; k < 4; ++k) ldmatrix_x4(rowS + px * 128u + (((2u * k + lk) ^ (px & 7u)) << 4), f[h][k]);
+            }
+            if (kx == 2) done_row = ring + 1u;
+            if (a == 0 && ky == 2 && kx == 2) { mbar_wait(&fullR[(ridx + 3) % kRows], ((ridx + 3) / kRows) & 1u); release_row(ridx + 3); }
+            if (++kx == 3) { kx = 0; if (++ky == 3) { ky = 0; ridx += 4; } }
+        };
+        auto mma = [&](const uint32_t (&f)[kH][4][4], bool first_of_tile) {
+            const uint32_t sb = m % kS;
+            mbar_wait(&fullB[sb], (m / kS) & 1u);
+            const uint64_t b_desc = make_desc_sw128(smem_u32(sB + sb * Cfg::kBSlot));
+            wgmma_fence();
+#pragma unroll
+            for (int h = 0; h < kH; ++h) fence_regs(acc[h]);
+#pragma unroll
+            for (uint32_t k = 0; k < 4; ++k)
+#pragma unroll
+                for (int h = 0; h < kH; ++h) wgmma_rs_row<N>(acc[h], f[h][k], b_desc + 2 * k);
+            wgmma_commit();
+#pragma unroll
+            for (int h = 0; h < kH; ++h) fence_regs(acc[h]);
+            if (done_row) { release_row(done_row - 1u); done_row = 0; }
+            if constexpr (GN) {
+                wgmma_wait<0>();
+                release_w(m);
+                if (threadIdx.x == 0 && m >= 1 && m - 1 + kS < total_steps) issue_w(m - 1 + kS);
+            } else {
+                wgmma_wait<1>();
+                if (!first_of_tile) release_w(m - 1);
+            }
+            ++m;
+        };
+
         for (uint32_t tile = tile0; tile < total_tiles; tile += tstep) {
             const uint32_t b = tile / tiles_per_img, y0 = (tile - b * tiles_per_img) * 2;
-            float acc0[64], acc1[64];
-#pragma unroll
-            for (int i = 0; i < 64; ++i) { acc0[i] = 0.0f; acc1[i] = 0.0f; }
-            for (uint32_t j = 0; j < KC; ++j) {
-                const uint32_t unused = ridx + (a == 0 ? 3u : 0u);
-                if (a == 1) { mbar_wait(&fullR[unused % kRwRows], (unused / kRwRows) & 1u); release_row(unused); }
-                for (uint32_t ky = 0; ky < 3; ++ky) {
-                    const uint32_t ring = ridx + ky + a;
-                    mbar_wait(&fullR[ring % kRwRows], (ring / kRwRows) & 1u);
-                    const uint32_t rowS = smem_u32(sR + (ring % kRwRows) * kRwRowSlot);
-                    for (uint32_t kx = 0; kx < 3; ++kx) {
-                        const uint32_t sb = m % kRwBStages;
-                        uint32_t af[2][4][4];
-#pragma unroll
-                        for (uint32_t h = 0; h < 2; ++h) {
-                            const uint32_t px = 64u * h + lrow + kx;
-#pragma unroll
-                            for (uint32_t k = 0; k < 4; ++k) ldmatrix_x4(rowS + px * 128u + (((2u * k + lk) ^ (px & 7u)) << 4), af[h][k]);
+#pragma unroll
+            for (int h = 0; h < kH; ++h)
+#pragma unroll
+                for (int i = 0; i < N / 2; ++i) acc[h][i] = 0.0f;
+            load_frags(af0);
+            if constexpr (GN) {
+                for (uint32_t s = 0;; ++s) {
+                    mma(af0, s == 0);
+                    if (s + 1 == steps_per_tile) break;
+                    load_frags(af0);
+                }
+            } else {
+                for (uint32_t s = 0;; s += 2) {
+                    mma(af0, s == 0);
+                    if (s + 1 == steps_per_tile) break;
+                    load_frags(af1);
+                    mma(af1, false);
+                    if (s + 2 == steps_per_tile) break;
+                    load_frags(af0);
+                }
+                wgmma_wait<0>();
+#pragma unroll
+                for (int h = 0; h < kH; ++h) fence_regs(acc[h]);
+                release_w(m - 1);
+            }
+            const size_t base = (((size_t)b * p.H + y0 + a) * W + wq * 16u + ((uint32_t)lane >> 2)) * N + 2u * cq;
+            const __half* res = p.residual ? p.residual + base : nullptr;
+            __half* out = p.out + base;
+            constexpr auto out_off = [](int i, int h, int hh) { return (64 * h + 8 * hh) * N + 8 * i; };
+            constexpr int kI = (GN ? 4 : 8) / kH;
+#pragma unroll
+            for (int i0 = 0; i0 < N / 8; i0 += kI) {
+                __half2 rv[kI][kH][2];
+                if (p.residual) {
+#pragma unroll
+                    for (int ii = 0; ii < kI; ++ii)
+#pragma unroll
+                        for (int h = 0; h < kH; ++h)
+#pragma unroll
+                            for (int hh = 0; hh < 2; ++hh) rv[ii][h][hh] = *reinterpret_cast<const __half2*>(res + out_off(i0 + ii, h, hh));
+                }
+#pragma unroll
+                for (int ii = 0; ii < kI; ++ii) {
+                    const int i = i0 + ii;
+                    const uint32_t ch = 8u * i + 2u * cq;
+                    const float b0 = sbias[ch], b1 = sbias[ch + 1];
+                    float su = 0.0f, sq = 0.0f;
+#pragma unroll
+                    for (int h = 0; h < kH; ++h) {
+#pragma unroll
+                        for (int hh = 0; hh < 2; ++hh) {
+                            float v0 = acc[h][4 * i + 2 * hh] + b0, v1 = acc[h][4 * i + 2 * hh + 1] + b1;
+                            if (p.residual) { const float2 r = __half22float2(rv[ii][h][hh]); v0 += r.x; v1 += r.y; }
+                            *reinterpret_cast<__half2*>(out + out_off(i, h, hh)) = __floats2half2_rn(v0, v1);
+                            su += v0 + v1; sq = fmaf(v0, v0, fmaf(v1, v1, sq));
                         }
-                        if (kx == 2) release_row(ring);
-                        mbar_wait(&fullB[sb], (m / kRwBStages) & 1u);
-                        const uint64_t b_desc = make_desc_sw128(smem_u32(sB + sb * kRwBSlot));
-                        wgmma_fence();
-                        fence_regs(acc0); fence_regs(acc1);
-#pragma unroll
-                        for (uint32_t k = 0; k < 4; ++k) {
-                            wgmma_rs_n128(acc0, af[0][k], b_desc + 2 * k, 1u);
-                            wgmma_rs_n128(acc1, af[1][k], b_desc + 2 * k, 1u);
-                        }
-                        wgmma_commit();
-                        wgmma_wait<0>();
-                        fence_regs(acc0); fence_regs(acc1);
-                        if (lane == 0) mbar_arrive(&emptyB[sb]);
-                        if (threadIdx.x == 0 && m >= 1 && m - 1 + kRwBStages < total_steps) issue_w(m - 1 + kRwBStages);
-                        ++m;
                     }
-                }
-                if (a == 0) { mbar_wait(&fullR[unused % kRwRows], (unused / kRwRows) & 1u); release_row(unused); }
-                ridx += 4;
-            }
-            const size_t pix0 = ((size_t)b * p.H + y0 + a) * kRwW;
-#pragma unroll
-            for (int i = 0; i < 16; ++i) {
-                const uint32_t ch = 8u * i + 2u * cq;
-                const float b0 = sbias[ch], b1 = sbias[ch + 1];
-                float su = 0.0f, sq = 0.0f;
-#pragma unroll
-                for (int h = 0; h < 2; ++h) {
-#pragma unroll
-                    for (int hh = 0; hh < 2; ++hh) {
-                        const size_t o = (pix0 + 64u * h + wq * 16u + ((uint32_t)lane >> 2) + 8u * hh) * kRwN + ch;
-                        float v0 = (h ? acc1 : acc0)[4 * i + 2 * hh] + b0, v1 = (h ? acc1 : acc0)[4 * i + 2 * hh + 1] + b1;
-                        if (p.residual) { const float2 r = __half22float2(*reinterpret_cast<const __half2*>(p.residual + o)); v0 += r.x; v1 += r.y; }
-                        *reinterpret_cast<__half2*>(p.out + o) = __floats2half2_rn(v0, v1);
-                        su += v0 + v1; sq = fmaf(v0, v0, fmaf(v1, v1, sq));
+                    if (p.qstats) {
+                        frag_quad_reduce(su, sq);
+                        if ((lane & ~2) == 0) { float* qa = qacc + (2 * i + (lane >> 1)) * 2; atomicAdd(qa, su); atomicAdd(qa + 1, sq); }
                     }
-                }
-                if (p.qstats) {
-                    frag_quad_reduce(su, sq);
-                    if ((lane & ~2) == 0) { float* qa = qacc + (2 * i + (lane >> 1)) * 2; atomicAdd(qa, su); atomicAdd(qa + 1, sq); }
                 }
             }
             if (p.qstats) {
                 asm volatile("bar.sync 1, 256;" ::: "memory");
-                if (threadIdx.x < 64) {
+                if (threadIdx.x < N / 2) {
                     const float val = qacc[threadIdx.x];
-                    if (val != 0.0f) atomicAdd(p.qstats + (size_t)b * 64 + threadIdx.x, val);
+                    if (val != 0.0f) atomicAdd(p.qstats + (size_t)b * (N / 2) + threadIdx.x, val);
                     qacc[threadIdx.x] = 0.0f;
                 }
                 asm volatile("bar.sync 1, 256;" ::: "memory");
@@ -250,14 +340,16 @@
 int make_map_4d_box(CUtensorMap* m, const void* base, uint64_t K, uint64_t e1, uint64_t e2, uint64_t e3, uint64_t s1, uint64_t s2, uint64_t s3,
                     uint32_t x1, uint32_t x2, uint32_t x3);
 
-template <bool GN>
-static int launch_row2(const CUtensorMap& mB, const ConvRowParams& p, int sms, cudaStream_t stream) {
+template <bool GN, int W, int N>
+static int launch_row2(const CUtensorMap& mB, const CUtensorMap& mX1, const CUtensorMap& mX2, const ConvRowParams& p, int sms, cudaStream_t stream) {
+    constexpr size_t kSmem = RowCfg<W, N>::kSmem;
     static DeviceOnce attr;
     if (attr.first()) {
-        SSDNERF_CUDA_OK(cudaFuncSetAttribute(k_conv_row2<GN>, cudaFuncAttributeMaxDynamicSharedMemorySize, (int)kRwSmem));
+        SSDNERF_CUDA_OK(cudaFuncSetAttribute(k_conv_row2<GN, W, N>, cudaFuncAttributeMaxDynamicSharedMemorySize, (int)kSmem));
     }
     const uint32_t total = p.B * (p.H / 2);
-    SSDNERF_CUDA_OK(launch_pdl(k_conv_row2<GN>, dim3(total < (uint32_t)sms ? total : (uint32_t)sms), dim3(kRwThreads), kRwSmem, stream, mB, p));
+    SSDNERF_CUDA_OK(launch_pdl(k_conv_row2<GN, W, N>, dim3(total < (uint32_t)sms ? total : (uint32_t)sms), dim3(kRwThreads), kSmem, stream,
+                               mB, mX1, mX2, p));
     SSDNERF_LAUNCH_OK();
     return 0;
 }
@@ -267,17 +359,24 @@
         (a->a2 && (((uintptr_t)a->a2 & 15u) || ((a->a2_strides[0] | a->a2_strides[1] | a->a2_strides[2]) & 15u))) ||
         ((uintptr_t)a->out & 3u) || ((uintptr_t)a->residual & 3u))
         return set_error_msg(SSDNERF_ERR_ARG, "gemm: row-pair convolution needs 16-byte aligned inputs and strides, 4-byte aligned output / residual");
+    const uint32_t W = a->d1, N = a->n;
     ConvRowParams p{};
     p.B = a->d3; p.H = a->d2;
     p.x1 = (const __half*)a->a1; p.C1 = a->k1;
     p.x2 = (const __half*)a->a2; p.C2 = a->a2 ? a->k2 : 0;
-    for (int i = 0; i < 3; ++i) { p.xs1[i] = (long long)(a->a1_strides[i] / 2); p.xs2[i] = a->a2 ? (long long)(a->a2_strides[i] / 2) : 0; }
     p.bias = a->bias_n; p.residual = (const __half*)a->residual; p.out = (__half*)a->out; p.qstats = a->qstats;
     const uint64_t ktot = (uint64_t)a->k1 + (a->a2 ? a->k2 : 0);
-    CUtensorMap mB;
+    CUtensorMap mB, mX1, mX2;
     if (int e = make_map_4d_box(&mB, a->b, ktot, a->n_rows_b ? a->n_rows_b : a->n, a->bx2 ? a->bx2 : 1, a->bx3 ? a->bx3 : 1, a->b_strides[0],
-                                a->b_strides[1], a->b_strides[2], kRwN, 1, 1)) return e;
-    return launch_row2<false>(mB, p, sms, stream);
+                                a->b_strides[1], a->b_strides[2], N, 1, 1)) return e;
+    if (int e = make_map_4d_box(&mX1, a->a1, a->k1, W, p.H, p.B, a->a1_strides[0], a->a1_strides[1], a->a1_strides[2], W + 2, 1, 1)) return e;
+    if (a->a2) {
+        if (int e = make_map_4d_box(&mX2, a->a2, a->k2, W, p.H, p.B, a->a2_strides[0], a->a2_strides[1], a->a2_strides[2], W + 2, 1, 1)) return e;
+    } else {
+        mX2 = mX1;
+    }
+    if (W == 64) return launch_row2<false, 64, 256>(mB, mX1, mX2, p, sms, stream);
+    return launch_row2<false, 128, 128>(mB, mX1, mX2, p, sms, stream);
 }
 
 }
@@ -296,19 +395,20 @@
     if (a->w_rows < 128) return set_error_msg(SSDNERF_ERR_ARG, "conv3x3_gn: packed weight needs >= 128 rows per tap");
     if (((uintptr_t)a->x1 | (uintptr_t)a->x2 | (uintptr_t)a->out | (uintptr_t)a->residual | (uintptr_t)a->w | (uintptr_t)a->coef_workspace) & 15u)
         return set_error_msg(SSDNERF_ERR_ARG, "conv3x3_gn: tensors must be 16-byte aligned");
+    constexpr uint32_t W = 128;
     ConvRowParams p{};
     p.B = a->B; p.H = a->H; p.x1 = (const __half*)a->x1; p.C1 = a->C1; p.x2 = (const __half*)a->x2; p.C2 = a->x2 ? a->C2 : 0;
-    p.xs1[0] = p.C1; p.xs1[1] = (long long)kRwW * p.C1; p.xs1[2] = (long long)p.H * kRwW * p.C1;
-    p.xs2[0] = p.C2; p.xs2[1] = (long long)kRwW * p.C2; p.xs2[2] = (long long)p.H * kRwW * p.C2;
+    p.xs1[0] = p.C1; p.xs1[1] = (long long)W * p.C1; p.xs1[2] = (long long)p.H * W * p.C1;
+    p.xs2[0] = p.C2; p.xs2[1] = (long long)W * p.C2; p.xs2[2] = (long long)p.H * W * p.C2;
     p.coef = (const float2*)a->coef_workspace; p.bias = a->bias; p.residual = (const __half*)a->residual; p.out = (__half*)a->out; p.qstats = a->qstats;
     int dev = 0, sms = 0;
     SSDNERF_CUDA_OK(cudaGetDevice(&dev));
     SSDNERF_CUDA_OK(cudaDeviceGetAttribute(&sms, cudaDevAttrMultiProcessorCount, dev));
-    SSDNERF_CUDA_OK(launch_pdl(k_gn_coef, dim3(a->B), dim3(128), 0, stream, a->q1, a->C1, a->x2 ? a->q2 : (const float*)nullptr, p.C2, a->H * 128u,
+    SSDNERF_CUDA_OK(launch_pdl(k_gn_coef, dim3(a->B), dim3(128), 0, stream, a->q1, a->C1, a->x2 ? a->q2 : (const float*)nullptr, p.C2, a->H * W,
                                a->gamma, a->beta, a->scale_shift, a->ss_batch_stride, a->eps, (float2*)a->coef_workspace));
     SSDNERF_LAUNCH_OK();
     CUtensorMap mB;
     if (int e = make_map_4d_box(&mB, a->w, C, a->w_rows, 9, 1, (uint64_t)C * 2, (uint64_t)a->w_rows * C * 2, (uint64_t)9 * a->w_rows * C * 2,
-                                kRwN, 1, 1)) return e;
-    return launch_row2<true>(mB, p, sms, stream);
-}
+                                128, 1, 1)) return e;
+    return launch_row2<true, 128, 128>(mB, mB, mB, p, sms, stream);
+}
diff --git a/ssdnerf_b200/csrc/conv_row_epilogue.cuh b/ssdnerf_b200/csrc/conv_row_epilogue.cuh
--- a/ssdnerf_b200/csrc/conv_row_epilogue.cuh
+++ b/ssdnerf_b200/csrc/conv_row_epilogue.cuh
@@ -2,8 +2,6 @@
 #include "common.cuh"
 
 namespace ssdnerf {
-
-constexpr int kRwW = 128, kRwN = 128;
 
 __device__ __forceinline__ void frag_quad_reduce(float& su, float& sq) {
     su += __shfl_xor_sync(0xffffffffu, su, 1); sq += __shfl_xor_sync(0xffffffffu, sq, 1);
diff --git a/ssdnerf_b200/csrc/gemm_tc.cu b/ssdnerf_b200/csrc/gemm_tc.cu
--- a/ssdnerf_b200/csrc/gemm_tc.cu
+++ b/ssdnerf_b200/csrc/gemm_tc.cu
@@ -337,11 +337,15 @@
     int dev = 0, sms = 0;
     SSDNERF_CUDA_OK(cudaGetDevice(&dev));
     SSDNERF_CUDA_OK(cudaDeviceGetAttribute(&sms, cudaDevAttrMultiProcessorCount, dev));
-    if (a->algo != 1 && a->taps == 9 && !a->tap_offsets && a_stride == 1 && a->d1 == 128 && a->b1 == 128 && a->b2 == 1 && a->b3 == 1 && a->n == 128 && !a->out_f32 && !a->b_batched &&
-        (a->d2 % 2) == 0 && a->alpha == 1.0f && (a->bn == 0 || a->bn == 128) && a->cluster <= 1 && a->so1 == 128 && a->so2 == 128 * 128 &&
-        a->so3 == (long long)a->d2 * 128 * 128 && (!a->qstats || a->stats_hw == 0) && (a->n_rows_b == 0 || a->n_rows_b >= 128))
+    const long long rw = a->d1, rn = a->n;
+    if (a->algo != 1 && a->taps == 9 && !a->tap_offsets && a_stride == 1 && ((rw == 128 && rn == 128) || (rw == 64 && rn == 256)) && a->b1 == rw &&
+        a->b3 == 1 && !a->out_f32 && !a->b_batched && (a->d2 % 2) == 0 && a->alpha == 1.0f && (a->bn == 0 || a->bn == rn) && a->cluster <= 1 &&
+        a->so1 == rn && a->so2 == rw * rn && a->so3 == (long long)a->d2 * rw * rn && (!a->qstats || a->stats_hw == 0) &&
+        (a->n_rows_b == 0 || a->n_rows_b >= rn))
         return ssdnerf::conv_row2_launch(a, sms, stream);
-    if (a->algo == 2) return set_error_msg(SSDNERF_ERR_ARG, "gemm: algo 2 (row-pair convolution) needs taps 9, 128-pixel rows, 128 output channels, fp16 output");
+    if (a->algo == 2)
+        return set_error_msg(SSDNERF_ERR_ARG, "gemm: algo 2 (row-pair convolution) needs taps 9 and 128-pixel rows with 128 output channels or "
+                                              "64-pixel rows with 256 output channels, fp16 output");
     int bn = (int)a->bn;
     if (!bn) {
         const uint32_t tiles_m = div_up(a->d1, a->b1) * div_up(a->d2, a->b2) * div_up(a->d3, a->b3);
diff --git a/ssdnerf_b200/csrc/tc_common.cuh b/ssdnerf_b200/csrc/tc_common.cuh
--- a/ssdnerf_b200/csrc/tc_common.cuh
+++ b/ssdnerf_b200/csrc/tc_common.cuh
@@ -118,6 +118,15 @@
         : "+f"(d[0]), "+f"(d[1]), "+f"(d[2]), "+f"(d[3]), "+f"(d[4]), "+f"(d[5]), "+f"(d[6]), "+f"(d[7]), "+f"(d[8]), "+f"(d[9]), "+f"(d[10]), "+f"(d[11]), "+f"(d[12]), "+f"(d[13]), "+f"(d[14]), "+f"(d[15]), "+f"(d[16]), "+f"(d[17]), "+f"(d[18]), "+f"(d[19]), "+f"(d[20]), "+f"(d[21]), "+f"(d[22]), "+f"(d[23]), "+f"(d[24]), "+f"(d[25]), "+f"(d[26]), "+f"(d[27]), "+f"(d[28]), "+f"(d[29]), "+f"(d[30]), "+f"(d[31]), "+f"(d[32]), "+f"(d[33]), "+f"(d[34]), "+f"(d[35]), "+f"(d[36]), "+f"(d[37]), "+f"(d[38]), "+f"(d[39]), "+f"(d[40]), "+f"(d[41]), "+f"(d[42]), "+f"(d[43]), "+f"(d[44]), "+f"(d[45]), "+f"(d[46]), "+f"(d[47]), "+f"(d[48]), "+f"(d[49]), "+f"(d[50]), "+f"(d[51]), "+f"(d[52]), "+f"(d[53]), "+f"(d[54]), "+f"(d[55]), "+f"(d[56]), "+f"(d[57]), "+f"(d[58]), "+f"(d[59]), "+f"(d[60]), "+f"(d[61]), "+f"(d[62]), "+f"(d[63])
         : "r"(a[0]), "r"(a[1]), "r"(a[2]), "r"(a[3]), "l"(b_desc), "r"(accumulate));
 }
+__device__ __forceinline__ void wgmma_rs_n256(float (&d)[128], const uint32_t (&a)[4], uint64_t b_desc, uint32_t accumulate) {
+    asm volatile(
+        "{\n\t.reg .pred p;\n\t"
+        "setp.ne.b32 p, %133, 0;\n\t"
+        "wgmma.mma_async.sync.aligned.m64n256k16.f32.f16.f16 "
+        "{%0, %1, %2, %3, %4, %5, %6, %7, %8, %9, %10, %11, %12, %13, %14, %15, %16, %17, %18, %19, %20, %21, %22, %23, %24, %25, %26, %27, %28, %29, %30, %31, %32, %33, %34, %35, %36, %37, %38, %39, %40, %41, %42, %43, %44, %45, %46, %47, %48, %49, %50, %51, %52, %53, %54, %55, %56, %57, %58, %59, %60, %61, %62, %63, %64, %65, %66, %67, %68, %69, %70, %71, %72, %73, %74, %75, %76, %77, %78, %79, %80, %81, %82, %83, %84, %85, %86, %87, %88, %89, %90, %91, %92, %93, %94, %95, %96, %97, %98, %99, %100, %101, %102, %103, %104, %105, %106, %107, %108, %109, %110, %111, %112, %113, %114, %115, %116, %117, %118, %119, %120, %121, %122, %123, %124, %125, %126, %127}, {%128, %129, %130, %131}, %132, p, 1, 1, 0;\n\t}"
+        : "+f"(d[0]), "+f"(d[1]), "+f"(d[2]), "+f"(d[3]), "+f"(d[4]), "+f"(d[5]), "+f"(d[6]), "+f"(d[7]), "+f"(d[8]), "+f"(d[9]), "+f"(d[10]), "+f"(d[11]), "+f"(d[12]), "+f"(d[13]), "+f"(d[14]), "+f"(d[15]), "+f"(d[16]), "+f"(d[17]), "+f"(d[18]), "+f"(d[19]), "+f"(d[20]), "+f"(d[21]), "+f"(d[22]), "+f"(d[23]), "+f"(d[24]), "+f"(d[25]), "+f"(d[26]), "+f"(d[27]), "+f"(d[28]), "+f"(d[29]), "+f"(d[30]), "+f"(d[31]), "+f"(d[32]), "+f"(d[33]), "+f"(d[34]), "+f"(d[35]), "+f"(d[36]), "+f"(d[37]), "+f"(d[38]), "+f"(d[39]), "+f"(d[40]), "+f"(d[41]), "+f"(d[42]), "+f"(d[43]), "+f"(d[44]), "+f"(d[45]), "+f"(d[46]), "+f"(d[47]), "+f"(d[48]), "+f"(d[49]), "+f"(d[50]), "+f"(d[51]), "+f"(d[52]), "+f"(d[53]), "+f"(d[54]), "+f"(d[55]), "+f"(d[56]), "+f"(d[57]), "+f"(d[58]), "+f"(d[59]), "+f"(d[60]), "+f"(d[61]), "+f"(d[62]), "+f"(d[63]), "+f"(d[64]), "+f"(d[65]), "+f"(d[66]), "+f"(d[67]), "+f"(d[68]), "+f"(d[69]), "+f"(d[70]), "+f"(d[71]), "+f"(d[72]), "+f"(d[73]), "+f"(d[74]), "+f"(d[75]), "+f"(d[76]), "+f"(d[77]), "+f"(d[78]), "+f"(d[79]), "+f"(d[80]), "+f"(d[81]), "+f"(d[82]), "+f"(d[83]), "+f"(d[84]), "+f"(d[85]), "+f"(d[86]), "+f"(d[87]), "+f"(d[88]), "+f"(d[89]), "+f"(d[90]), "+f"(d[91]), "+f"(d[92]), "+f"(d[93]), "+f"(d[94]), "+f"(d[95]), "+f"(d[96]), "+f"(d[97]), "+f"(d[98]), "+f"(d[99]), "+f"(d[100]), "+f"(d[101]), "+f"(d[102]), "+f"(d[103]), "+f"(d[104]), "+f"(d[105]), "+f"(d[106]), "+f"(d[107]), "+f"(d[108]), "+f"(d[109]), "+f"(d[110]), "+f"(d[111]), "+f"(d[112]), "+f"(d[113]), "+f"(d[114]), "+f"(d[115]), "+f"(d[116]), "+f"(d[117]), "+f"(d[118]), "+f"(d[119]), "+f"(d[120]), "+f"(d[121]), "+f"(d[122]), "+f"(d[123]), "+f"(d[124]), "+f"(d[125]), "+f"(d[126]), "+f"(d[127])
+        : "r"(a[0]), "r"(a[1]), "r"(a[2]), "r"(a[3]), "l"(b_desc), "r"(accumulate));
+}
 __device__ __forceinline__ void wgmma_ss_n256(float (&d)[128], uint64_t a_desc, uint64_t b_desc, uint32_t accumulate) {
     asm volatile(
         "{\n\t.reg .pred p;\n\t"
```

After: 80.02 million (median of 6 runs). About the same (-0.1%).
